# Wuziyi616/CFUN

Measured on AMD Instinct MI355X. Metric: volumes/sec fwd+bwd, 256x256x128 8-class CT, higher is better.
Workload: dtype f32; 1 GPU; cfg2: 256x256x128 CT, stage 'finetune', 4 positive + 8 negative RoIs, U-Net b=20, 96x96x96 crops -> 192x192x192 masks, 6 losses incl. 3-D Sobel edge loss, fwd+bwd; parallelism=single GPU

## Files before the change

cfun_amd/_lib.py:

```python
import ctypes as C
import os

import torch

_HERE = os.path.dirname(os.path.abspath(__file__))
DEFAULT_LIB = os.path.join(_HERE, "libcfun_hip.so")

ACT_NONE, ACT_RELU, ACT_LRELU = 0, 1, 2
ALGO_AUTO, ALGO_DIRECT, ALGO_MFMA = 0, 1, 2
ALGO_WINO = 4
ALGO_WINO2 = 5
TILE_G16, TILE_G8 = 0x100, 0x200


class ConvParams(C.Structure):
    _fields_ = [(n, C.c_int32) for n in ("N", "Di", "Hi", "Wi", "Ci", "Do", "Ho", "Wo", "Co", "CoP", "CiP",
                                         "kd", "kh", "kw", "stride", "pd", "ph", "pw", "up2", "act")] + \
               [("slope", C.c_float)] + \
               [(n, C.c_int32) for n in ("scale_mode", "has_shift", "res_mode", "res_up2", "d2s", "d2s_cq", "tap_skip", "algo",
                                         "w_prepared")]


class ConvFusion(C.Structure):
    _fields_ = [("in_stats", C.c_void_p), ("in_act", C.c_int32), ("in_slope", C.c_float), ("out_stats", C.c_void_p),
                ("out_eps", C.c_float)]


FUSE_OUT_STATS, FUSE_IN_NORM, FUSE_IN_NORM_WGRAD = 1, 2, 4


class WeightJob(C.Structure):
    _fields_ = [("w", C.c_void_p), ("fwd", C.c_void_p), ("dgrad", C.c_void_p), ("co_idx", C.c_void_p), ("ci_idx", C.c_void_p),
                ("Co", C.c_int32), ("Ci", C.c_int32), ("T", C.c_int32), ("src_ci", C.c_int32), ("fwd_kind", C.c_int32),
                ("dgrad_kind", C.c_int32), ("block_begin", C.c_uint32), ("reserved", C.c_int32)]


WOP_NONE = 0

_P = C.c_void_p
_I = C.c_int32
_L = C.c_int64
_F = C.c_float
_Z = C.c_size_t
_PP = C.POINTER(ConvParams)
_PF = C.POINTER(ConvFusion)

_SIGNATURES = {
    "cfun_version": (C.c_int, []),
    "cfun_error_string": (C.c_char_p, [C.c_int]),
    "cfun_conv3d_fwd_workspace_bytes": (_Z, [_PP]),
    "cfun_conv3d_fwd_kernel": (_I, [_PP]),
    "cfun_conv3d_wino_plan": (C.c_int, [_PP, C.POINTER(C.c_int32)]),
    "cfun_conv3d_fwd": (C.c_int, [_P, _P, _P, _P, _P, _P, _PP, _P, _Z, _P]),
    "cfun_conv3d_fused_support": (C.c_int, [_PP]),
    "cfun_conv3d_fwd_fused_workspace_bytes": (_Z, [_PP, _PF]),
    "cfun_conv3d_fwd_fused": (C.c_int, [_P, _P, _P, _P, _P, _P, _PP, _PF, _P, _Z, _P]),
    "cfun_conv3d_bwd_weight_fused": (C.c_int, [_P, _P, _P, _I, _PP, _PF, _P, _Z, _P]),
    "cfun_conv3d_bwd_data_workspace_bytes": (_Z, [_PP]),
    "cfun_conv3d_bwd_data": (C.c_int, [_P, _P, _P, _PP, _P, _Z, _P]),
    "cfun_conv3d_bwd_weight_workspace_bytes": (_Z, [_PP]),
    "cfun_conv3d_bwd_weight": (C.c_int, [_P, _P, _P, _PP, _P, _Z, _P]),
    "cfun_conv3d_bwd_weight_oidhw": (C.c_int, [_P, _P, _P, _PP, _P, _Z, _P]),
    "cfun_act_bwd": (C.c_int, [_P, _P, _P, _P, _L, _I, _L, _I, _F, _I, _P]),
    "cfun_channel_sum_workspace_bytes": (_Z, [_L, _I]),
    "cfun_channel_sum": (C.c_int, [_P, _P, _L, _I, _P, _Z, _P]),
    "cfun_fc_workspace_bytes": (_Z, [_I, _I, _I]),
    "cfun_fc_fwd": (C.c_int, [_P, _P, _P, _P, _P, _I, _I, _I, _I, _P, _Z, _P]),
    "cfun_fc_bwd_weight": (C.c_int, [_P, _P, _P, _I, _I, _I, _P]),
    "cfun_fc_bwd_weight_max_rows": (_I, [_I]),
    "cfun_fc_bwd_data": (C.c_int, [_P, _P, _P, _I, _I, _I, _P]),
    "cfun_lrelu_fwd": (C.c_int, [_P, _P, _L, _F, _P]),
    "cfun_lrelu_bwd": (C.c_int, [_P, _P, _P, _L, _F, _P]),
    "cfun_add": (C.c_int, [_P, _P, _P, _L, _P]),
    "cfun_lrelu_bwd_add": (C.c_int, [_P, _P, _P, _P, _L, _I, _L, _F, _P]),
    "cfun_instnorm_lrelu_bwd_add": (C.c_int, [_P, _P, _P, _P, _P, _I, _L, _I, _L, _F, _P, _Z, _P]),
    "cfun_upsample2_bwd": (C.c_int, [_P, _P, _I, _I, _I, _I, _I, _P]),
    "cfun_instnorm_workspace_bytes": (_Z, [_I, _L, _I]),
    "cfun_instnorm_stats": (C.c_int, [_P, _P, _I, _L, _I, _F, _P, _Z, _P]),
    "cfun_instnorm_lrelu_fwd": (C.c_int, [_P, _P, _P, _I, _L, _I, _F, _P]),
    "cfun_instnorm_lrelu_bwd": (C.c_int, [_P, _P, _P, _P, _I, _L, _I, _F, _P, _Z, _P]),
    "cfun_instnorm_lrelu_fwd_strided": (C.c_int, [_P, _P, _P, _I, _L, _I, _L, _F, _P]),
    "cfun_instnorm_lrelu_bwd_strided": (C.c_int, [_P, _P, _P, _P, _I, _L, _I, _L, _F, _P, _Z, _P]),
    "cfun_instnorm_bwd_means": (C.c_int, [_P, _P, _P, _P, _I, _L, _I, _L, _F, _P, _Z, _P]),
    "cfun_instnorm_lrelu_bwd_apply": (C.c_int, [_P, _P, _P, _P, _P, _I, _L, _I, _L, _F, _P]),
    "cfun_lrelu_fwd_strided": (C.c_int, [_P, _P, _L, _I, _L, _L, _F, _P]),
    "cfun_lrelu_bwd_strided": (C.c_int, [_P, _P, _P, _L, _I, _L, _F, _P]),
    "cfun_maxpool2_fwd": (C.c_int, [_P, _P, _P, _I, _I, _I, _I, _I, _P]),
    "cfun_maxpool2_bwd": (C.c_int, [_P, _P, _P, _I, _I, _I, _I, _I, _P]),
    "cfun_roi_align3d_fwd": (C.c_int, [_P, _P, _P, _P, _I, _I, _I, _I, _I, _I, _I, _I, _P]),
    "cfun_roi_align3d_bwd": (C.c_int, [_P, _P, _P, _I, _I, _I, _I, _I, _I, _I, _I, _P]),
    "cfun_roi_align3d_slab_fwd": (C.c_int, [_P, _P, _P, _P, _I, _I, _I, _I, _I, _I, _I, _I, _I, _I, _P]),
    "cfun_roi_align3d_slab_bwd": (C.c_int, [_P, _P, _P, _I, _I, _I, _I, _I, _I, _I, _I, _I, _I, _P]),
    "cfun_nms3d_workspace_bytes": (_Z, [_I]),
    "cfun_nms3d": (C.c_int, [_P, _P, _I, _F, _I, _P, _P, _P, _Z, _P]),
    "cfun_softmax_fwd": (C.c_int, [_P, _P, _L, _I, _P]),
    "cfun_softmax_bwd": (C.c_int, [_P, _P, _P, _L, _I, _P]),
    "cfun_loss_workspace_bytes": (_Z, [_L]),
    "cfun_softmax_ce_fwd": (C.c_int, [_P, _P, _P, _L, _I, _P, _Z, _P]),
    "cfun_softmax_ce_bwd": (C.c_int, [_P, _P, _P, _P, _L, _I, _P]),
    "cfun_edge_loss_fwd": (C.c_int, [_P, _P, _P, _I, _I, _I, _I, _I, _P, _Z, _P]),
    "cfun_edge_loss_bwd_workspace_bytes": (_Z, [_I, _I, _I, _I, _I]),
    "cfun_edge_loss_bwd": (C.c_int, [_P, _P, _P, _P, _I, _I, _I, _I, _I, _P, _Z, _P]),
    "cfun_mask_losses_bwd": (C.c_int, [_P, _P, _P, _P, _P, _I, _I, _I, _I, _I, _P, _Z, _P]),
    "cfun_edge_loss_fwd_save": (C.c_int, [_P, _P, _P, _P, _I, _I, _I, _I, _I, _P, _Z, _P]),
    "cfun_mask_losses_bwd_saved": (C.c_int, [_P, _P, _P, _P, _P, _P, _I, _I, _I, _I, _I, _P]),
    "cfun_mask_fused_workspace_bytes": (_Z, []),
    "cfun_mask_fused_supported": (C.c_int, [_I, _I, _I, _I, _I]),
    "cfun_mask_fused_fwd": (C.c_int, [_P, _P, _P, _P, _P, _I, _I, _I, _I, _I, _P, _Z, _P]),
    "cfun_mask_fused_u_bytes": (_Z, [_I, _I, _I, _I, _I]),
    "cfun_mask_fused_bwd": (C.c_int, [_P, _P, _P, _P, _P, _I, _I, _I, _I, _I, _P]),
    "cfun_mask_target_labels": (C.c_int, [_P, _P, _P, _I, _I, _I, _I, _I, _I, _I, _P]),
    "cfun_ce_weighted_workspace_bytes": (_Z, []),
    "cfun_softmax_ce_weighted_fwd": (C.c_int, [_P, _P, _P, _P, _P, _L, _I, _P, _Z, _P]),
    "cfun_softmax_ce_weighted_bwd": (C.c_int, [_P, _P, _P, _P, _P, _P, _L, _I, _P]),
    "cfun_edge_raw_dc_bytes": (_Z, [_I, _I, _I, _I, _I]),
    "cfun_edge_raw_fwd": (C.c_int, [_P, _P, _P, _P, _I, _I, _I, _I, _I, _P, _Z, _P]),
    "cfun_edge_raw_bwd": (C.c_int, [_P, _P, _P, _I, _I, _I, _I, _I, _P]),
    "cfun_unmold_argmax": (C.c_int, [_P, _P, _I, _I, _I, _I, _I, _I, _I, _P, _P]),
    "cfun_unmold_overlap": (C.c_int, [_P, _P, _I, _P, _P, _I, _I, _I, _I, _I, _I, _I, _P]),
    "cfun_sumsq_partials_count": (C.c_int32, []),
    "cfun_sumsq_partials": (C.c_int, [_P, C.c_int64, _P, _P]),
    "cfun_norm_finalize": (C.c_int, [_P, _I, _P, _P]),
    "cfun_sgd_momentum_step": (C.c_int, [_P, _P, _P, C.c_int64, C.c_float, C.c_float, C.c_float, C.c_float, _P, _I, _P]),
    "cfun_weight_pack": (C.c_int, [_P, _P, _I, _I, _I, _P]),
    "cfun_weight_pack_transpose": (C.c_int, [_P, _P, _I, _I, _I, _P]),
    "cfun_weight_pack_both": (C.c_int, [_P, _P, _P, _I, _I, _I, _P]),
    "cfun_fold_up2_fwd": (C.c_int, [_P, _P, _I, _I, _I, _I, _P]),
    "cfun_fold_up2_bwd": (C.c_int, [_P, _P, _I, _I, _I, _I, _P]),
    "cfun_weight_prepare_kinds": (C.c_int, [_PP, C.POINTER(C.c_int32), C.POINTER(C.c_size_t)]),
    "cfun_weight_prepare_plan": (C.c_int, [C.POINTER(WeightJob), _I, C.POINTER(C.c_int64)]),
    "cfun_weight_prepare": (C.c_int, [_P, _I, _L, _P]),
    "cfun_weight_unpack": (C.c_int, [_P, _P, _I, _I, _I, _P]),
    "cfun_halo_pack": (C.c_int, [_P, _P, _I, _I, _I, _I, _I, _I, _I, _P]),
    "cfun_halo_unpack": (C.c_int, [_P, _P, _I, _I, _I, _I, _I, _I, _I, _P]),
    "cfun_resize3d": (C.c_int, [_P, _P, _P, _P, _P, _P, _P, _I, _P, _P]),
}

EXPORTS = tuple(_SIGNATURES)

_D = C.c_double
SAMPLE_SIGNATURES = {
    "cfun_sample_workspace_bytes": (_Z, [_I, _I, _I, _I, _I]),
    "cfun_sample_rotate_bbox": (C.c_int, [_P, _P, _P, _P, _P, _D, _D, _I, _P, _P, _P, _P, _P, _P, _Z, _P]),
    "cfun_sample_rpn_targets": (C.c_int, [_P, _I, _P, _I, _P, _I, _P, _D, _D, _P, _P, _P, _P, _Z, _P]),
}
SAMPLE_EXPORTS = tuple(SAMPLE_SIGNATURES)

TILE_SIGNATURES = {
    "cfun_conv3d_fwd_tile": (C.c_int, [_PP, C.POINTER(C.c_int32)]),
}
TILE_EXPORTS = tuple(TILE_SIGNATURES)

EVAL_SIGNATURES = {
    "cfun_seg_confusion_workspace_bytes": (_Z, [_I, _I, _I, _I]),
    "cfun_seg_confusion": (C.c_int, [_P, _P, _I, _P, _P, _I, _P, _P, _Z, _P]),
}
EVAL_EXPORTS = tuple(EVAL_SIGNATURES)

CC_CLASS, CC_FOREGROUND = 0, 1
CC_SIGNATURES = {
    "cfun_cc_workspace_bytes": (_Z, [_I, _I, _I, _I]),
    "cfun_cc_label": (C.c_int, [_P, _P, _I, _I, _P, _P, _Z, _P]),
    "cfun_cc_filter": (C.c_int, [_P, _P, _P, _I, _I, _I, _L, _P, _P, _P, _Z, _P]),
}
CC_EXPORTS = tuple(CC_SIGNATURES)

_lib = None
_lib_path = None
_is_emulator = False


def lib_path():
    return os.environ.get("CFUN_LIB_PATH") or DEFAULT_LIB


def load():
    global _lib, _lib_path, _is_emulator
    path = lib_path()
    if _lib is not None and _lib_path == path:
        return _lib
    if not os.path.exists(path):
        raise RuntimeError(
            "cfun_amd: %s not found -- the HIP library is required (no CPU fallback). Build it with "
            "`make -C cfun_amd/csrc -j8` or `python -c 'import __graft_entry__ as g; g.build()'`." % path)
    lib = C.CDLL(path)
    for name, (res, args) in list(_SIGNATURES.items()) + list(SAMPLE_SIGNATURES.items()) + list(TILE_SIGNATURES.items()) + \
            list(EVAL_SIGNATURES.items()) + list(CC_SIGNATURES.items()):
        fn = getattr(lib, name)
        fn.restype = res
        fn.argtypes = args
    _lib, _lib_path = lib, path
    _is_emulator = os.path.basename(path).startswith("libcfun_emu")
    return lib


def is_emulator():
    load()
    return _is_emulator


def check(rc, what):
    if rc != 0:
        msg = load().cfun_error_string(rc)
        raise RuntimeError("cfun_amd: %s failed (%d): %s" % (what, rc, msg.decode() if msg else "?"))


def ptr(t):
    if t is None:
        return None
    if not t.is_contiguous():
        raise RuntimeError("cfun_amd: kernel argument must be contiguous, got strides %s" % (t.stride(),))
    if not t.is_cuda and not is_emulator():
        raise RuntimeError("cfun_amd: CPU tensor passed to a HIP kernel (there is no CPU fallback)")
    return t.data_ptr()


def stream(t):
    if t.is_cuda:
        return torch.cuda.current_stream(t.device).cuda_stream
    return None


def workspace(nbytes, like):
    return torch.empty(max(int(nbytes), 256), dtype=torch.uint8, device=like.device)
```

cfun_amd/csrc/conv3d.hip:

```cpp
#include <stdlib.h>

#include "conv3d_mfma.h"
#include "../../include/cfun_tile.h"

int cfun_conv_fwd_direct(const float*, const float*, const float*, const float*, const float*, float*,
                         const CfunConv3dParams*, hipStream_t);
int cfun_conv_bwd_data_direct(const float*, const float*, float*, const CfunConv3dParams*, hipStream_t);
int cfun_conv_bwd_weight_direct(const float*, const float*, CfunWgradDst, const CfunConv3dParams*, void*, size_t, hipStream_t);
size_t cfun_direct_wgrad_ws(const CfunConv3dParams*);
int cfun_wgrad_finish(const float*, CfunWgradDst, const CfunConv3dParams*, int, hipStream_t);
int cfun_wgrad_zero(CfunWgradDst, const CfunConv3dParams*, hipStream_t);
int cfun_conv_stem_supported(const CfunConv3dParams*);
int cfun_conv_stem_fwd(const float*, const float*, const float*, const float*, float*, const CfunConv3dParams*, hipStream_t);
int cfun_conv_pointwise_supported(const CfunConv3dParams*);
int cfun_conv_pointwise_in_supported(const CfunConv3dParams*);
int cfun_conv_pointwise_fwd(const float*, const float*, const float*, const float*, const float*, float*,
                            const CfunConv3dParams*, const float*, int, float, hipStream_t);
int cfun_wino_supported(const CfunConv3dParams*);
size_t cfun_wino_workspace_bytes(const CfunConv3dParams*);
int cfun_wino_s2d_dgrad_supported(const CfunConv3dParams*, const CfunConv3dParams*);
int cfun_wino_fwd(const float*, const float*, int, int, const float*, const float*, const float*, float*,
                  const CfunConv3dParams*, void*, size_t, const cfun_mfma::ConvMode*, int, hipStream_t);
int cfun_wino_is_2d(const CfunConv3dParams*);
int cfun_wino_geom(const CfunConv3dParams*);
int cfun_wino_stat_slots(const CfunConv3dParams*, size_t);
int cfun_stats_finalize(const double* part, float* stats, int N, int slots, int C, int64_t V, float eps, int slot_minor, hipStream_t st);
int cfun_wino_wgrad_supported(const CfunConv3dParams*);
size_t cfun_wino_wgrad_workspace_bytes(const CfunConv3dParams*);
int cfun_wino_wgrad(const float*, const float*, float*, const CfunConv3dParams*, int*, hipStream_t);
int cfun_wgrad_c1_supported(const CfunConv3dParams*);
size_t cfun_wgrad_c1_ws(const CfunConv3dParams*);
int cfun_wgrad_c1(const float*, const float*, CfunWgradDst, const CfunConv3dParams*, void*, size_t, hipStream_t);

namespace {

typedef int (*FwdFn)(int, const float*, const float*, const float*, const float*, const float*, float*,
                     const CfunConv3dParams&, const cfun_mfma::ConvMode&, void*, size_t, hipStream_t);
typedef size_t (*FwdWsFn)(int, const CfunConv3dParams&, const cfun_mfma::ConvMode&);
typedef void (*PlanFn)(const CfunConv3dParams&, int, cfun_mfma::WgPlan*);
typedef int (*WgFn)(const float*, const float*, float*, const CfunConv3dParams&, const cfun_mfma::WgPlan&, hipStream_t);

struct Shape {
  int kd, kh, kw, s;
  FwdFn fwd;
  FwdWsFn fwd_ws;
  PlanFn plan;
  WgFn wgrad;
  int max_nsub;
  FwdFn fwd8;
  FwdWsFn fwd_ws8;
};

#define SHAPE(NAME, KD, KH, KW, S, MAXN) \
  { KD, KH, KW, S, cfun_mfma_fwd_##NAME, cfun_mfma_fwd_ws_##NAME, cfun_mfma_wgrad_plan_##NAME, cfun_mfma_wgrad_##NAME, MAXN, \
    nullptr, nullptr }
#define SHAPE_G8(NAME, KD, KH, KW, S, MAXN) \
  { KD, KH, KW, S, cfun_mfma_fwd_##NAME, cfun_mfma_fwd_ws_##NAME, cfun_mfma_wgrad_plan_##NAME, cfun_mfma_wgrad_##NAME, MAXN, \
    cfun_mfma_fwd_g8_##NAME, cfun_mfma_fwd_ws_g8_##NAME }
const Shape kShapes[] = {
    SHAPE_G8(k333s1, 3, 3, 3, 1, 5), SHAPE_G8(k333s2, 3, 3, 3, 2, 5), SHAPE(k111s1, 1, 1, 1, 1, 5),
    SHAPE(k111s2, 1, 1, 1, 2, 5), SHAPE(k133s1, 1, 3, 3, 1, 5), SHAPE(k311s1, 3, 1, 1, 1, 5),
    SHAPE(k555s1, 5, 5, 5, 1, 1), SHAPE_G8(k222s1, 2, 2, 2, 1, 5),
};

const Shape* find_shape(int kd, int kh, int kw, int s) {
  for (const Shape& sh : kShapes)
    if (sh.kd == kd && sh.kh == kh && sh.kw == kw && sh.s == s) return &sh;
  return nullptr;
}

using cfun_mfma::ConvMode;
const ConvMode kPlain = {0, 0, 0, 0, 0, nullptr, 0, 0.f, nullptr, 0};

int pick_nsub_parity(int cqp, int max_nsub) {
  for (int n = max_nsub; n >= 1; --n)
    if (cqp % (16 * n) == 0) return n;
  return 0;
}

int pick_nsub(int co, int max_nsub) {
  int best = 1, best_pad = 1 << 30;
  for (int n = 1; n <= max_nsub; ++n) {
    const int nt = 16 * n;
    const int pad = (co + nt - 1) / nt * nt;
    if (pad <= best_pad) { best_pad = pad; best = n; }
  }
  return best;
}

bool standard_dims(const CfunConv3dParams* p) {
  const int sh = p->up2 ? 1 : 0;
  return (((p->Di << sh) + 2 * p->pd - p->kd) / p->stride + 1) == p->Do &&
         (((p->Hi << sh) + 2 * p->ph - p->kh) / p->stride + 1) == p->Ho &&
         (((p->Wi << sh) + 2 * p->pw - p->kw) / p->stride + 1) == p->Wo;
}

bool valid_params(const CfunConv3dParams* p) {
  if (!p) return false;
  if (p->N < 0 || p->Ci <= 0 || p->Co <= 0 || p->kd <= 0 || p->kh <= 0 || p->kw <= 0) return false;
  if (p->stride != 1 && p->stride != 2) return false;
  if (p->CoP < p->Co || (p->CoP & 15) || p->CiP < p->Ci || (p->CiP & 15)) return false;
  if (!standard_dims(p)) return false;
  if (p->d2s) {
    if ((p->Co & 7) || p->up2 || p->d2s_cq < 0 || p->d2s_cq > (p->Co >> 3)) return false;
    if (p->tap_skip && !(p->kd == 3 && p->kh == 3 && p->kw == 3 && p->stride == 1)) return false;
  } else if (p->tap_skip || p->d2s_cq) {
    return false;
  } else if (p->res_mode && p->res_up2 && ((p->Do | p->Ho | p->Wo) & 1)) {
    return false;
  }
  return true;
}

const Shape* mfma_shape(const CfunConv3dParams* p) {
  if ((p->Ci & 3) || (p->Co & 3)) return nullptr;
  if (p->d2s) {
    const int cqp = p->Co >> 3, cq = p->d2s_cq > 0 ? p->d2s_cq : cqp;
    if ((cqp & 3) || (cq & 3)) return nullptr;
    if (p->tap_skip && pick_nsub_parity(cqp, 5) == 0) return nullptr;
  }
  const Shape* s = find_shape(p->kd, p->kh, p->kw, p->stride);
  if (!s) return nullptr;
  if (p->Co > 16 * s->max_nsub && s->max_nsub == 1) return nullptr;
  return s;
}

int tile_geom_knob() {
  static int v = -2;
  if (v == -2) {
    const char* e = getenv("CFUN_TILE_GEOM");
    v = !e ? -1 : atoi(e) == 16 ? 0 : atoi(e) == 8 ? 1 : -1;
  }
  return v;
}

bool tile_geom_rule(const CfunConv3dParams* p) {
  using cfun_mfma::cdiv;
  const int64_t g16 = (int64_t)cdiv(p->Ho, 4) * 4 * cdiv(p->Wo, 16) * 16, g8 = (int64_t)cdiv(p->Ho, 8) * 8 * cdiv(p->Wo, 8) * 8;
  return g8 < g16;
}

bool make_dgrad_params(const CfunConv3dParams* p, CfunConv3dParams* q) {
  if (p->stride != 1 || !standard_dims(p)) return false;
  const int sh = p->up2 ? 1 : 0;
  *q = *p;
  q->Di = p->Do; q->Hi = p->Ho; q->Wi = p->Wo; q->Ci = p->Co;
  q->Do = p->Di << sh; q->Ho = p->Hi << sh; q->Wo = p->Wi << sh; q->Co = p->Ci;
  q->CoP = p->CiP; q->CiP = p->CoP;
  q->pd = p->kd - 1 - p->pd; q->ph = p->kh - 1 - p->ph; q->pw = p->kw - 1 - p->pw;
  if (q->pd < 0 || q->ph < 0 || q->pw < 0) return false;
  q->up2 = 0; q->act = CFUN_ACT_NONE; q->scale_mode = 0; q->has_shift = 0; q->res_mode = 0; q->res_up2 = 0;
  q->d2s = 0; q->d2s_cq = 0; q->tap_skip = 0; q->w_prepared = 0;
  return true;
}

bool use_folded_s2_dgrad(const CfunConv3dParams* p) {
  return CFUN_ALGO_OF(p->algo) != CFUN_ALGO_DIRECT && p->stride == 2 && !p->up2 && p->kd == 3 && p->kh == 3 && p->kw == 3 &&
         p->pd == 1 && p->ph == 1 && p->pw == 1 && !((p->Di | p->Hi | p->Wi) & 1) && !(p->Ci & 3) && !(p->Co & 3) &&
         p->Di == 2 * p->Do && p->Hi == 2 * p->Ho && p->Wi == 2 * p->Wo;
}

__global__ void __launch_bounds__(256)
k_fold_s2_dgrad_weights(const float* __restrict__ wpT, float* __restrict__ wd, int Ci, int Co, int CiP, int CoPd) {
  const int64_t total = (int64_t)8 * Co * CoPd;
  const int64_t i = (int64_t)blockIdx.x * 256 + threadIdx.x;
  if (i >= total) return;
  const int col = (int)(i % CoPd);
  const int co = (int)((i / CoPd) % Co);
  const int tap = (int)(i / ((int64_t)CoPd * Co));
  float v = 0.f;
  if (col < 8 * Ci) {
    const int q = col / Ci, ci = col - q * Ci;
    const int par[3] = {q >> 2, (q >> 1) & 1, q & 1}, off[3] = {tap >> 2, (tap >> 1) & 1, tap & 1};
    int t[3];
    bool ok = true;
    for (int d = 0; d < 3; ++d) {
      if (par[d] == 0) { t[d] = 1; ok = ok && off[d] == 0; }
      else t[d] = off[d] == 0 ? 2 : 0;
    }
    if (ok) v = wpT[((int64_t)((t[0] * 3 + t[1]) * 3 + t[2]) * Co + co) * CiP + ci];
  }
  wd[i] = v;
}

CfunConv3dParams folded_s2_params(const CfunConv3dParams* p) {
  CfunConv3dParams q = *p;
  q.Di = p->Do; q.Hi = p->Ho; q.Wi = p->Wo; q.Ci = p->Co;
  q.Do = p->Do; q.Ho = p->Ho; q.Wo = p->Wo; q.Co = 8 * p->Ci;
  q.CoP = (8 * p->Ci + 15) / 16 * 16; q.CiP = p->CoP;
  q.kd = q.kh = q.kw = 2; q.stride = 1; q.pd = q.ph = q.pw = 0;
  q.up2 = 0; q.act = CFUN_ACT_NONE; q.scale_mode = 0; q.has_shift = 0; q.res_mode = 0; q.res_up2 = 0; q.d2s = 1;
  q.d2s_cq = 0; q.tap_skip = 0; q.w_prepared = 0;
  return q;
}

int wgrad_max_nsub(const Shape* s) {
  static int cap = -1;
  if (cap < 0) {
    const char* e = getenv("CFUN_WGRAD_MAX_NSUB");
    cap = e ? atoi(e) : 5;
    if (cap < 1 || cap > 5) cap = 5;
  }
  return s->max_nsub < cap ? s->max_nsub : cap;
}

int wgrad_nsub(const CfunConv3dParams* p, const Shape* s) {
  if (p->d2s && p->tap_skip) {
    const int cqp = p->Co >> 3, mx = wgrad_max_nsub(s);
    const int tiles = (cqp + 16 * mx - 1) / (16 * mx);
    return (cqp + 16 * tiles - 1) / (16 * tiles);
  }
  return pick_nsub(p->CoP, wgrad_max_nsub(s));
}

bool use_mfma_dgrad(const CfunConv3dParams* p, CfunConv3dParams* q, const Shape** s) {
  if (CFUN_ALGO_OF(p->algo) == CFUN_ALGO_DIRECT) return false;
  if (!make_dgrad_params(p, q)) return false;
  *s = mfma_shape(q);
  return *s != nullptr;
}

__global__ void __launch_bounds__(256)
k_splitk_finish(const float4* __restrict__ partial, int ksplit, const float* __restrict__ scale,
                const float* __restrict__ shift, const float* __restrict__ res, float4* __restrict__ y,
                CfunConv3dParams p, int64_t total4) {
  const int C4 = p.Co >> 2;
  for (int64_t i = (int64_t)blockIdx.x * 256 + threadIdx.x; i < total4; i += (int64_t)gridDim.x * 256) {
    float4 a = partial[i];
    for (int k = 1; k < ksplit; ++k) {
      const float4 b = partial[(int64_t)k * total4 + i];
      a.x += b.x; a.y += b.y; a.z += b.z; a.w += b.w;
    }
    const int64_t v = i / C4;
    const int co = (int)(i - v * C4) * 4;
    if (p.scale_mode) {
      const int64_t n = v / ((int64_t)p.Do * p.Ho * p.Wo);
      const float4 s4 = *reinterpret_cast<const float4*>(scale + (p.scale_mode == 2 ? n * p.Co : 0) + co);
      a.x *= s4.x; a.y *= s4.y; a.z *= s4.z; a.w *= s4.w;
    }
    if (p.has_shift) {
      const float4 t = *reinterpret_cast<const float4*>(shift + co);
      a.x += t.x; a.y += t.y; a.z += t.z; a.w += t.w;
    }
    if (p.res_mode) {
      int64_t rv = v;
      if (p.res_up2) {
        int64_t t = v;
        const int ox = (int)(t % p.Wo); t /= p.Wo;
        const int oy = (int)(t % p.Ho); t /= p.Ho;
        const int oz = (int)(t % p.Do);
        const int64_t n = t / p.Do;
        rv = ((n * (p.Do >> 1) + (oz >> 1)) * (p.Ho >> 1) + (oy >> 1)) * (p.Wo >> 1) + (ox >> 1);
      }
      const float4 t4 = *reinterpret_cast<const float4*>(res + rv * p.Co + co);
      a.x += t4.x; a.y += t4.y; a.z += t4.z; a.w += t4.w;
    }
    a.x = cfun_apply_act(a.x, p.act, p.slope); a.y = cfun_apply_act(a.y, p.act, p.slope);
    a.z = cfun_apply_act(a.z, p.act, p.slope); a.w = cfun_apply_act(a.w, p.act, p.slope);
    y[i] = a;
  }
}

__global__ void __launch_bounds__(256)
k_splitk_finish_stats(const float4* __restrict__ partial, int ksplit, const float* __restrict__ scale,
                      const float* __restrict__ shift, const float* __restrict__ res, float4* __restrict__ y,
                      CfunConv3dParams p, int64_t V, int lanes, double* __restrict__ part) {
  __shared__ double sm[256 * 8];
  const int C4 = p.Co >> 2, tid = threadIdx.x;
  const int cg = tid % C4, vl = tid / C4, n = blockIdx.y, co = cg * 4;
  const int64_t total4 = (int64_t)p.N * V * C4;
  double acc[2][4] = {{0.0, 0.0, 0.0, 0.0}, {0.0, 0.0, 0.0, 0.0}};
  if (vl < lanes) {
    float4 s4 = make_float4(1.f, 1.f, 1.f, 1.f), t4 = make_float4(0.f, 0.f, 0.f, 0.f);
    if (p.scale_mode) s4 = *reinterpret_cast<const float4*>(scale + (p.scale_mode == 2 ? n * p.Co : 0) + co);
    if (p.has_shift) t4 = *reinterpret_cast<const float4*>(shift + co);
#pragma unroll 4
    for (int64_t vv = (int64_t)blockIdx.x * lanes + vl; vv < V; vv += (int64_t)gridDim.x * lanes) {
      const int64_t v = (int64_t)n * V + vv, i = v * C4 + cg;
      float4 a = partial[i];
      for (int k = 1; k < ksplit; ++k) {
        const float4 b = partial[(int64_t)k * total4 + i];
        a.x += b.x; a.y += b.y; a.z += b.z; a.w += b.w;
      }
      if (p.scale_mode) { a.x *= s4.x; a.y *= s4.y; a.z *= s4.z; a.w *= s4.w; }
      if (p.has_shift) { a.x += t4.x; a.y += t4.y; a.z += t4.z; a.w += t4.w; }
      if (p.res_mode) {
        int64_t rv = v;
        if (p.res_up2) {
          int64_t t = vv;
          const int ox = (int)(t % p.Wo); t /= p.Wo;
          const int oy = (int)(t % p.Ho);
          const int oz = (int)(t / p.Ho);
          rv = (((int64_t)n * (p.Do >> 1) + (oz >> 1)) * (p.Ho >> 1) + (oy >> 1)) * (p.Wo >> 1) + (ox >> 1);
        }
        const float4 r4 = *reinterpret_cast<const float4*>(res + rv * p.Co + co);
        a.x += r4.x; a.y += r4.y; a.z += r4.z; a.w += r4.w;
      }
      a.x = cfun_apply_act(a.x, p.act, p.slope); a.y = cfun_apply_act(a.y, p.act, p.slope);
      a.z = cfun_apply_act(a.z, p.act, p.slope); a.w = cfun_apply_act(a.w, p.act, p.slope);
      y[i] = a;
      acc[0][0] += a.x; acc[0][1] += a.y; acc[0][2] += a.z; acc[0][3] += a.w;
      acc[1][0] += (double)a.x * a.x; acc[1][1] += (double)a.y * a.y; acc[1][2] += (double)a.z * a.z; acc[1][3] += (double)a.w * a.w;
    }
  }
#pragma unroll
  for (int q = 0; q < 2; ++q)
#pragma unroll
    for (int j = 0; j < 4; ++j) sm[(tid * 2 + q) * 4 + j] = acc[q][j];
  __syncthreads();
  if (vl == 0) {
    for (int l = 1; l < lanes; ++l) {
      const int t2 = l * C4 + cg;
#pragma unroll
      for (int q = 0; q < 2; ++q)
#pragma unroll
        for (int j = 0; j < 4; ++j) acc[q][j] += sm[(t2 * 2 + q) * 4 + j];
    }
    double* out = part + ((int64_t)n * gridDim.x + blockIdx.x) * 2 * p.Co;
#pragma unroll
    for (int q = 0; q < 2; ++q)
#pragma unroll
      for (int j = 0; j < 4; ++j) out[(int64_t)q * p.Co + co + j] = acc[q][j];
  }
}

int splitk_stats_blocks(const CfunConv3dParams* p, int* lanes_out) {
  const int C4 = p->Co >> 2;
  if ((p->Co & 3) || C4 > 256 || C4 < 1) return 0;
  const int lanes = 256 / C4;
  const int64_t V = (int64_t)p->Do * p->Ho * p->Wo;
  int64_t want = (4096 + p->N - 1) / (p->N > 0 ? p->N : 1);
  int64_t maxb = (V + (int64_t)lanes * 4 - 1) / ((int64_t)lanes * 4);
  if (maxb < 1) maxb = 1;
  if (lanes_out) *lanes_out = lanes;
  return (int)(want < maxb ? want : maxb);
}

}

int cfun_splitk_stat_slots(const CfunConv3dParams* p) { return splitk_stats_blocks(p, nullptr); }

int cfun_tile_geom(const CfunConv3dParams* p, int g8_exists) {
  if (!g8_exists || (p->algo & CFUN_ALGO_TILE_G16)) return 0;
  if (p->algo & CFUN_ALGO_TILE_G8) return 1;
  if (tile_geom_knob() >= 0) return tile_geom_knob();
  return g8_exists == 1 && tile_geom_rule(p) ? 1 : 0;
}

int cfun_splitk_finish(const float* partial, int ksplit, const float* scale, const float* shift, const float* res,
                       float* y, const CfunConv3dParams* p, double* stat_part, hipStream_t st) {
  if (stat_part) {
    int lanes = 0;
    const int blocks = splitk_stats_blocks(p, &lanes);
    if (blocks <= 0) return CFUN_EINVAL;
    hipLaunchKernelGGL(k_splitk_finish_stats, dim3((unsigned)blocks, (unsigned)p->N), dim3(256), 0, st, (const float4*)partial,
                       ksplit, scale, shift, res, (float4*)y, *p, (int64_t)p->Do * p->Ho * p->Wo, lanes, stat_part);
    CFUN_LAUNCH_CHECK();
    return CFUN_OK;
  }
  const int64_t total4 = (int64_t)p->N * p->Do * p->Ho * p->Wo * (p->Co >> 2);
  int64_t blocks = (total4 + 255) / 256;
  if (blocks > 2048) blocks = 2048;
  hipLaunchKernelGGL(k_splitk_finish, dim3((unsigned)blocks), dim3(256), 0, st, (const float4*)partial, ksplit, scale, shift,
                     res, (float4*)y, *p, total4);
  CFUN_LAUNCH_CHECK();
  return CFUN_OK;
}

extern "C" {

int cfun_version(void) { return CFUN_VERSION; }

const char* cfun_error_string(int code) {
  switch (code) {
    case CFUN_OK: return "ok";
    case CFUN_EINVAL: return "cfun: invalid argument or unsupported shape";
    case CFUN_EWORKSPACE: return "cfun: workspace too small";
    case CFUN_EALIGN: return "cfun: pointer not 16-byte aligned";
    default: return code > 0 ? hipGetErrorString((hipError_t)code) : "cfun: unknown error";
  }
}

static int pick_tile(const Shape* s, int co, bool per_parity) {
  const bool rem_ok = (s->kd == 3 && s->kh == 3 && s->kw == 3) || (s->kd == 1 && s->kh == 1 && s->kw == 1 && s->s == 1);
  if (rem_ok && s->max_nsub > 1) {
    if (co == 20) return 1 + 8 * 1;
    if (co == 8 && s->kd == 3) return 0 + 8 * 2;
  }
  return per_parity ? pick_nsub_parity(co, s->max_nsub) : pick_nsub(co, s->max_nsub);
}

static void fwd_mode(const CfunConv3dParams* p, const Shape* s, ConvMode* md, int* nsub) {
  *md = kPlain;
  *nsub = pick_tile(s, p->Co, false);
  if (p->d2s && p->tap_skip) {
    md->tap_skip = 1;
    *nsub = pick_tile(s, p->Co >> 3, true);
  }
}

static bool g8_loses_wave(const Shape* s, const ConvMode& md, int nsub) {
  if (s->kd == 2) return nsub == 1;
  if (s->s == 2) return nsub == 1 || nsub == 4 || nsub == 0 + 8 * 2;
  if (md.tap_skip == 1 || md.in_s2d) return false;
  return nsub == 3 || nsub == 4 || nsub == 5 || nsub == 1 + 8 * 1;
}

static bool g8_no_gain(const CfunConv3dParams* p, const Shape* s, const ConvMode& md) {
  return (s->kd == 2 || md.tap_skip == 1) && (int64_t)p->Do * p->Ho * p->Wo <= 6 * 6 * 6;
}

static int mfma_geom(const CfunConv3dParams* p, const Shape* s, const ConvMode& md, int nsub) {
  const bool has = s->fwd8 && nsub != 2 + 8 * 2 && (!md.in_s2d || (md.tap_skip == 2 && nsub < 8));
  return cfun_tile_geom(p, !has ? 0 : (g8_loses_wave(s, md, nsub) || g8_no_gain(p, s, md)) ? 2 : 1);
}

size_t cfun_conv3d_fwd_workspace_bytes(const CfunConv3dParams* p) {
  if (!valid_params(p)) return 0;
  const Shape* s = CFUN_ALGO_OF(p->algo) == CFUN_ALGO_DIRECT ? nullptr : mfma_shape(p);
  if (!s) return 256;
  ConvMode md;
  int nsub;
  fwd_mode(p, s, &md, &nsub);
  size_t need = (mfma_geom(p, s, md, nsub) ? s->fwd_ws8 : s->fwd_ws)(nsub, *p, md);
  if (cfun_wino_supported(p) && cfun_wino_workspace_bytes(p) > need) need = cfun_wino_workspace_bytes(p);
  return cfun_align_up(need + 256, 256);
}

int cfun_conv3d_fwd_kernel(const CfunConv3dParams* p);

int cfun_conv3d_fwd_tile(const CfunConv3dParams* p, int32_t out[3]) {
  if (!out || !valid_params(p)) return CFUN_EINVAL;
  const int k = cfun_conv3d_fwd_kernel(p);
  if (k != CFUN_KERNEL_MFMA && k != CFUN_KERNEL_WINO) return CFUN_EINVAL;
  int g;
  if (k == CFUN_KERNEL_WINO) {
    g = cfun_wino_geom(p);
  } else {
    ConvMode md;
    int nsub;
    const Shape* s = mfma_shape(p);
    fwd_mode(p, s, &md, &nsub);
    g = mfma_geom(p, s, md, nsub);
  }
  out[0] = 4; out[1] = g ? 8 : 4; out[2] = g ? 8 : 16;
  return CFUN_OK;
}

int cfun_conv3d_fwd_kernel(const CfunConv3dParams* p) {
  if (!valid_params(p)) return CFUN_EINVAL;
  if (CFUN_ALGO_OF(p->algo) == CFUN_ALGO_AUTO && cfun_conv_pointwise_supported(p)) return CFUN_KERNEL_POINTWISE;
  if (CFUN_ALGO_OF(p->algo) != CFUN_ALGO_DIRECT && mfma_shape(p)) return cfun_wino_supported(p) ? CFUN_KERNEL_WINO : CFUN_KERNEL_MFMA;
  if (CFUN_ALGO_OF(p->algo) != CFUN_ALGO_DIRECT && CFUN_ALGO_OF(p->algo) != CFUN_ALGO_MFMA && cfun_conv_stem_supported(p)) return CFUN_KERNEL_STEM;
  return CFUN_KERNEL_DIRECT;
}

static int conv_fwd_impl(const float* x, const float* wp, const float* scale, const float* shift, const float* res,
                         float* y, const CfunConv3dParams* p, const ConvMode* fz, void* ws, size_t ws_bytes,
                         int* stat_slots, cfun_stream_t stream) {
  if (!valid_params(p)) return CFUN_EINVAL;
  if ((p->scale_mode && !scale) || (p->has_shift && !shift) || (p->res_mode && !res)) return CFUN_EINVAL;
  if (p->scale_mode < 0 || p->scale_mode > 2 || p->res_mode < 0 || p->res_mode > 1) return CFUN_EINVAL;
  const bool fused = fz && (fz->in_stats || fz->in_act || fz->out_part);
  if (CFUN_ALGO_OF(p->algo) == CFUN_ALGO_AUTO && cfun_conv_pointwise_supported(p) && cfun_aligned16(x) && cfun_aligned16(y)) {
    if (fused && (fz->out_part || !cfun_conv_pointwise_in_supported(p))) return CFUN_EINVAL;
    return cfun_conv_pointwise_fwd(x, wp, scale, shift, res, y, p, fused ? fz->in_stats : nullptr, fused ? fz->in_act : 0,
                                   fused ? fz->in_slope : 0.f, cfun_st(stream));
  }
  const Shape* s = CFUN_ALGO_OF(p->algo) == CFUN_ALGO_DIRECT ? nullptr : mfma_shape(p);
  if (s) {
    if (!cfun_aligned16(x) || !cfun_aligned16(wp) || !cfun_aligned16(y) || (scale && !cfun_aligned16(scale)) ||
        (shift && !cfun_aligned16(shift)) || (res && !cfun_aligned16(res)))
      return CFUN_EALIGN;
    ConvMode md;
    int nsub;
    fwd_mode(p, s, &md, &nsub);
    if (fused) { md.in_stats = fz->in_stats; md.in_act = fz->in_act; md.in_slope = fz->in_slope; md.out_part = fz->out_part; }
    if (ws && !cfun_aligned16(ws)) return CFUN_EALIGN;
    const bool prepared = (p->w_prepared & 1) != 0;
    if (ws && cfun_wino_supported(p) && ws_bytes >= cfun_wino_workspace_bytes(p)) {
      if (md.in_stats || md.in_act) return CFUN_EINVAL;
      if (stat_slots) *stat_slots = cfun_wino_stat_slots(p, ws_bytes);
      return cfun_wino_fwd(x, wp, 0, 0, scale, shift, res, y, p, ws, ws_bytes, &md, prepared, cfun_st(stream));
    }
    if (prepared && cfun_wino_supported(p)) return CFUN_EWORKSPACE;
    const int geom = mfma_geom(p, s, md, nsub);
    if (stat_slots) *stat_slots = cfun_mfma::fwd_stat_slots(nsub, geom, *p, md, ws ? ws_bytes : 0);
    return (geom ? s->fwd8 : s->fwd)(nsub, x, wp, scale, shift, res, y, *p, md, ws, ws ? ws_bytes : 0, cfun_st(stream));
  }
  if (fused) return CFUN_EINVAL;
  if (CFUN_ALGO_OF(p->algo) == CFUN_ALGO_MFMA) return CFUN_EINVAL;
  if (CFUN_ALGO_OF(p->algo) != CFUN_ALGO_DIRECT && cfun_conv_stem_supported(p) && cfun_aligned16(y))
    return cfun_conv_stem_fwd(x, wp, scale, shift, y, p, cfun_st(stream));
  return cfun_conv_fwd_direct(x, wp, scale, shift, res, y, p, cfun_st(stream));
}

int cfun_conv3d_fwd(const float* x, const float* wp, const float* scale, const float* shift, const float* res,
                    float* y, const CfunConv3dParams* p, void* ws, size_t ws_bytes, cfun_stream_t stream) {
  return conv_fwd_impl(x, wp, scale, shift, res, y, p, nullptr, ws, ws_bytes, nullptr, stream);
}

static bool wgrad_takes_prologue(const CfunConv3dParams* p);

int cfun_conv3d_fused_support(const CfunConv3dParams* p) {
  if (!valid_params(p) || CFUN_ALGO_OF(p->algo) == CFUN_ALGO_DIRECT || !mfma_shape(p)) return 0;
  const int wg = wgrad_takes_prologue(p) ? CFUN_FUSE_IN_NORM_WGRAD : 0;
  if (CFUN_ALGO_OF(p->algo) == CFUN_ALGO_AUTO && cfun_conv_pointwise_supported(p))
    return cfun_conv_pointwise_in_supported(p) ? (CFUN_FUSE_IN_NORM | wg) : 0;
  const int st = (p->Co >> 2) <= 256 ? CFUN_FUSE_OUT_STATS : 0;
  if (cfun_wino_supported(p)) return st;
  return st | CFUN_FUSE_IN_NORM | wg;
}

static size_t stat_part_bytes(const CfunConv3dParams* p) {
  using cfun_mfma::cdiv;
  const int t16 = cdiv(p->Do, 4) * cdiv(p->Ho, 4) * cdiv(p->Wo, 16), t8 = cdiv(p->Do, 4) * cdiv(p->Ho, 8) * cdiv(p->Wo, 8);
  const int tiles = (t16 > t8 ? t16 : t8) * (p->d2s ? 8 : 1);
  const int sk = cfun_splitk_stat_slots(p);
  const int cy = p->d2s ? (p->d2s_cq > 0 ? p->d2s_cq : (p->Co >> 3)) : p->Co;
  return cfun_align_up((size_t)p->N * (tiles > sk ? tiles : sk) * 2 * cy * sizeof(double), 256);
}

size_t cfun_conv3d_fwd_fused_workspace_bytes(const CfunConv3dParams* p, const CfunConvFusion* f) {
  const size_t main_bytes = cfun_conv3d_fwd_workspace_bytes(p);
  if (!main_bytes || !f || !f->out_stats) return main_bytes;
  return main_bytes + stat_part_bytes(p);
}

int cfun_conv3d_fwd_fused(const float* x, const float* wp, const float* scale, const float* shift, const float* res,
                          float* y, const CfunConv3dParams* p, const CfunConvFusion* f, void* ws, size_t ws_bytes,
                          cfun_stream_t stream) {
  if (!f || (!f->in_stats && !f->in_act && !f->out_stats))
    return conv_fwd_impl(x, wp, scale, shift, res, y, p, nullptr, ws, ws_bytes, nullptr, stream);
  const int have = cfun_conv3d_fused_support(p);
  const int want = (f->out_stats ? CFUN_FUSE_OUT_STATS : 0) | ((f->in_stats || f->in_act) ? CFUN_FUSE_IN_NORM : 0);
  if ((want & have) != want) return CFUN_EINVAL;
  if (f->in_act != CFUN_ACT_NONE && (f->in_act != CFUN_ACT_LRELU || f->in_slope < 0.f || f->in_slope > 1.f)) return CFUN_EINVAL;
  ConvMode fz = kPlain;
  fz.in_stats = f->in_stats;
  fz.in_act = (f->in_stats || f->in_act) ? CFUN_ACT_LRELU : CFUN_ACT_NONE;
  fz.in_slope = f->in_act == CFUN_ACT_LRELU ? f->in_slope : 1.f;
  const size_t main_bytes = cfun_conv3d_fwd_workspace_bytes(p);
  if (f->out_stats) {
    if (!ws || !cfun_aligned16(ws) || ws_bytes < main_bytes + stat_part_bytes(p)) return CFUN_EWORKSPACE;
    fz.out_part = (double*)((char*)ws + main_bytes);
  }
  int slots = 0;
  const int rc = conv_fwd_impl(x, wp, scale, shift, res, y, p, &fz, ws, f->out_stats ? main_bytes : ws_bytes, &slots, stream);
  if (rc || !f->out_stats) return rc;
  if (slots == 0) return CFUN_EINVAL;
  const int cy = p->d2s ? (p->d2s_cq > 0 ? p->d2s_cq : (p->Co >> 3)) : p->Co;
  return cfun_stats_finalize(fz.out_part, f->out_stats, p->N, slots < 0 ? -slots : slots, cy,
                             (int64_t)p->Do * p->Ho * p->Wo * (p->d2s ? 8 : 1), f->out_eps, slots > 0, cfun_st(stream));
}

int cfun_weight_prepare_kinds(const CfunConv3dParams* p, int32_t kinds[2], size_t bytes[2]) {
  if (!kinds || !bytes) return CFUN_EINVAL;
  kinds[0] = kinds[1] = CFUN_WOP_NONE;
  bytes[0] = bytes[1] = 0;
  if (!valid_params(p)) return CFUN_EINVAL;
  const int T = p->kd * p->kh * p->kw;
  if (T > 27) return CFUN_OK;
  kinds[0] = CFUN_WOP_PACK;
  bytes[0] = (size_t)T * p->Ci * p->CoP * sizeof(float);
  const bool pointwise = CFUN_ALGO_OF(p->algo) == CFUN_ALGO_AUTO && cfun_conv_pointwise_supported(p);
  if (!pointwise && CFUN_ALGO_OF(p->algo) != CFUN_ALGO_DIRECT && mfma_shape(p) && cfun_wino_supported(p)) {
    const int twod = cfun_wino_is_2d(p);
    kinds[0] = twod ? CFUN_WOP_WINO2 : CFUN_WOP_WINO1;
    bytes[0] = (size_t)(twod ? 48 : 36) * p->Ci * p->CoP * sizeof(float);
  }
  kinds[1] = CFUN_WOP_PACKT;
  bytes[1] = (size_t)T * p->Co * p->CiP * sizeof(float);
  CfunConv3dParams q;
  const Shape* s;
  if (use_folded_s2_dgrad(p)) {
    kinds[1] = CFUN_WOP_S2FOLD;
    bytes[1] = (size_t)8 * p->Co * ((8 * p->Ci + 15) / 16 * 16) * sizeof(float);
  } else if (use_mfma_dgrad(p, &q, &s) && !p->up2 &&
             (p->d2s ? cfun_wino_s2d_dgrad_supported(p, &q) : cfun_wino_supported(&q))) {
    const int twod = cfun_wino_is_2d(&q);
    kinds[1] = twod ? CFUN_WOP_WINO2_T : CFUN_WOP_WINO1_T;
    bytes[1] = (size_t)(twod ? 48 : 36) * p->Co * p->CiP * sizeof(float);
  }
  return CFUN_OK;
}

size_t cfun_conv3d_bwd_data_workspace_bytes(const CfunConv3dParams* p) {
  if (!valid_params(p)) return 0;
  CfunConv3dParams q;
  const Shape* s;
  if (use_folded_s2_dgrad(p)) return cfun_align_up((size_t)8 * p->Co * ((8 * p->Ci + 15) / 16 * 16) * sizeof(float), 256);
  if (use_mfma_dgrad(p, &q, &s)) {
    if (p->up2) return cfun_align_up((size_t)q.N * q.Do * q.Ho * q.Wo * q.Co * sizeof(float), 256);
    ConvMode md = kPlain;
    md.flip = 1;
    if (p->d2s) { md.in_s2d = 1; md.in_cqp = p->Co >> 3; md.in_cq = p->d2s_cq > 0 ? p->d2s_cq : md.in_cqp; }
    const int nsub = pick_tile(s, q.Co, false);
    if (p->d2s) md.tap_skip = p->tap_skip ? 2 : 0;
    size_t need = (mfma_geom(&q, s, md, nsub) ? s->fwd_ws8 : s->fwd_ws)(nsub, q, md);
    if ((p->d2s ? cfun_wino_s2d_dgrad_supported(p, &q) : cfun_wino_supported(&q)) && cfun_wino_workspace_bytes(&q) > need)
      need = cfun_wino_workspace_bytes(&q);
    return cfun_align_up(need + 256, 256);
  }
  return 256;
}

int cfun_conv3d_bwd_data(const float* g, const float* wpT, float* dx, const CfunConv3dParams* p, void* ws,
                         size_t ws_bytes, cfun_stream_t stream) {
  if (!valid_params(p)) return CFUN_EINVAL;
  CfunConv3dParams q;
  const Shape* s;
  const bool prepared = (p->w_prepared & 2) != 0;
  if (use_folded_s2_dgrad(p)) {
    if (!cfun_aligned16(g) || !cfun_aligned16(wpT) || !cfun_aligned16(dx) || !cfun_aligned16(ws)) return CFUN_EALIGN;
    if (ws_bytes < cfun_conv3d_bwd_data_workspace_bytes(p)) return CFUN_EWORKSPACE;
    q = folded_s2_params(p);
    const float* wd = wpT;
    if (!prepared) {
      const int64_t nw = (int64_t)8 * p->Co * q.CoP;
      hipLaunchKernelGGL(k_fold_s2_dgrad_weights, dim3((unsigned)((nw + 255) / 256)), dim3(256), 0, cfun_st(stream), wpT,
                         (float*)ws, p->Ci, p->Co, p->CiP, q.CoP);
      CFUN_LAUNCH_CHECK();
      wd = (const float*)ws;
    }
    const Shape* s2 = find_shape(2, 2, 2, 1);
    const int nsub = pick_nsub(q.Co, s2->max_nsub);
    return (mfma_geom(&q, s2, kPlain, nsub) ? s2->fwd8 : s2->fwd)(nsub, g, wd, nullptr, nullptr, nullptr, dx, q, kPlain, nullptr, 0,
                                                                   cfun_st(stream));
  }
  if (use_mfma_dgrad(p, &q, &s)) {
    if (!cfun_aligned16(g) || !cfun_aligned16(wpT) || !cfun_aligned16(dx)) return CFUN_EALIGN;
    const int nsub = pick_tile(s, q.Co, false);
    ConvMode md = kPlain;
    md.flip = 1;
    if (p->d2s) {
      md.in_s2d = 1;
      md.in_cqp = p->Co >> 3;
      md.in_cq = p->d2s_cq > 0 ? p->d2s_cq : md.in_cqp;
      md.tap_skip = p->tap_skip ? 2 : 0;
    }
    const bool wino = !p->up2 && (p->d2s ? cfun_wino_s2d_dgrad_supported(p, &q) : cfun_wino_supported(&q));
    if (wino && cfun_aligned16(ws) && ws_bytes >= cfun_wino_workspace_bytes(&q))
      return cfun_wino_fwd(g, wpT, 1, p->d2s ? (p->Co >> 3) : 0, nullptr, nullptr, nullptr, dx, &q, ws, ws_bytes, nullptr,
                           prepared, cfun_st(stream));
    if (wino && prepared) return CFUN_EWORKSPACE;
    const FwdFn fwd = mfma_geom(&q, s, md, nsub) ? s->fwd8 : s->fwd;
    if (!p->up2) return fwd(nsub, g, wpT, nullptr, nullptr, nullptr, dx, q, md, ws, cfun_aligned16(ws) ? ws_bytes : 0, cfun_st(stream));
    if (ws_bytes < cfun_conv3d_bwd_data_workspace_bytes(p) || !cfun_aligned16(ws)) return CFUN_EWORKSPACE;
    const int rc = fwd(nsub, g, wpT, nullptr, nullptr, nullptr, (float*)ws, q, md, nullptr, 0, cfun_st(stream));
    if (rc) return rc;
    return cfun_upsample2_bwd((const float*)ws, dx, p->N, p->Di, p->Hi, p->Wi, p->Ci, stream);
  }
  return cfun_conv_bwd_data_direct(g, wpT, dx, p, cfun_st(stream));
}

static bool wgrad_mfma_fits(const CfunConv3dParams* p) {
  const int64_t lim = (int64_t)1 << 31;
  const int64_t go = (int64_t)p->N * p->Do * p->Ho * p->Wo * p->Co;
  return (int64_t)p->N * p->Di * p->Hi * p->Wi * p->Ci < lim && go < lim;
}

size_t cfun_conv3d_bwd_weight_workspace_bytes(const CfunConv3dParams* p) {
  if (!valid_params(p)) return 0;
  if (CFUN_ALGO_OF(p->algo) != CFUN_ALGO_DIRECT && cfun_wgrad_c1_supported(p)) return cfun_align_up(cfun_wgrad_c1_ws(p), 256);
  const Shape* s = (CFUN_ALGO_OF(p->algo) == CFUN_ALGO_DIRECT || !wgrad_mfma_fits(p)) ? nullptr : mfma_shape(p);
  if (s && cfun_wino_wgrad_supported(p)) return cfun_align_up(cfun_wino_wgrad_workspace_bytes(p), 256);
  if (s) {
    cfun_mfma::WgPlan w;
    s->plan(*p, wgrad_nsub(p, s), &w);
    return cfun_align_up((size_t)w.nchunks * w.kslots * p->kd * p->kh * p->kw * p->Ci * p->CoP * sizeof(float), 256);
  }
  return cfun_align_up(cfun_direct_wgrad_ws(p), 256);
}

static bool wgrad_takes_prologue(const CfunConv3dParams* p) {
  if (CFUN_ALGO_OF(p->algo) == CFUN_ALGO_DIRECT || !wgrad_mfma_fits(p) || !mfma_shape(p)) return false;
  return !cfun_wgrad_c1_supported(p) && !cfun_wino_wgrad_supported(p);
}

static int bwd_weight_any(const float* x, const float* g, CfunWgradDst dst, const CfunConv3dParams* p,
                          const CfunConvFusion* f, void* ws, size_t ws_bytes, cfun_stream_t stream) {
  if (!valid_params(p)) return CFUN_EINVAL;
  const bool pro = f && (f->in_stats || f->in_act);
  if (pro && !wgrad_takes_prologue(p)) return CFUN_EINVAL;
  if (CFUN_ALGO_OF(p->algo) != CFUN_ALGO_DIRECT && cfun_wgrad_c1_supported(p) && (int64_t)p->N * p->Do * p->Ho * p->Wo > 0) {
    if (!cfun_aligned16(g) || !cfun_aligned16(ws)) return CFUN_EALIGN;
    return cfun_wgrad_c1(x, g, dst, p, ws, ws_bytes, cfun_st(stream));
  }
  const Shape* s = (CFUN_ALGO_OF(p->algo) == CFUN_ALGO_DIRECT || !wgrad_mfma_fits(p)) ? nullptr : mfma_shape(p);
  if (s) {
    if (!cfun_aligned16(x) || !cfun_aligned16(g)) return CFUN_EALIGN;
    if (ws_bytes < cfun_conv3d_bwd_weight_workspace_bytes(p)) return CFUN_EWORKSPACE;
    if (cfun_wino_wgrad_supported(p)) {
      if (!cfun_aligned16(ws)) return CFUN_EALIGN;
      int nparts = 0;
      const int rc = cfun_wino_wgrad(x, g, (float*)ws, p, &nparts, cfun_st(stream));
      if (rc) return rc;
      return cfun_wgrad_finish((const float*)ws, dst, p, nparts, cfun_st(stream));
    }
    cfun_mfma::WgPlan w;
    s->plan(*p, wgrad_nsub(p, s), &w);
    if (pro) {
      if (f->in_act != CFUN_ACT_NONE && (f->in_act != CFUN_ACT_LRELU || f->in_slope < 0.f || f->in_slope > 1.f)) return CFUN_EINVAL;
      w.in_stats = f->in_stats; w.in_act = CFUN_ACT_LRELU; w.in_slope = f->in_act == CFUN_ACT_LRELU ? f->in_slope : 1.f;
    }
    if (w.ntiles == 0) return cfun_wgrad_zero(dst, p, cfun_st(stream));
    const int rc = s->wgrad(x, g, (float*)ws, *p, w, cfun_st(stream));
    if (rc) return rc;
    return cfun_wgrad_finish((const float*)ws, dst, p, w.nchunks * w.kslots, cfun_st(stream));
  }
  if (CFUN_ALGO_OF(p->algo) == CFUN_ALGO_MFMA) return CFUN_EINVAL;
  return cfun_conv_bwd_weight_direct(x, g, dst, p, ws, ws_bytes, cfun_st(stream));
}

int cfun_conv3d_bwd_weight(const float* x, const float* g, float* dwp, const CfunConv3dParams* p, void* ws,
                           size_t ws_bytes, cfun_stream_t stream) {
  return bwd_weight_any(x, g, CfunWgradDst{dwp, 0}, p, nullptr, ws, ws_bytes, stream);
}

int cfun_conv3d_bwd_weight_oidhw(const float* x, const float* g, float* dw, const CfunConv3dParams* p, void* ws,
                                 size_t ws_bytes, cfun_stream_t stream) {
  return bwd_weight_any(x, g, CfunWgradDst{dw, 1}, p, nullptr, ws, ws_bytes, stream);
}

int cfun_conv3d_bwd_weight_fused(const float* x, const float* g, float* dw, int32_t oidhw, const CfunConv3dParams* p,
                                 const CfunConvFusion* f, void* ws, size_t ws_bytes, cfun_stream_t stream) {
  return bwd_weight_any(x, g, CfunWgradDst{dw, oidhw ? 1 : 0}, p, f, ws, ws_bytes, stream);
}

}
```

cfun_amd/csrc/conv3d_mfma.h:

```cpp
#pragma once
#include <type_traits>

#include "common.h"

typedef float f32x4 __attribute__((ext_vector_type(4)));

int cfun_splitk_finish(const float* partial, int ksplit, const float* scale, const float* shift, const float* res,
                       float* y, const CfunConv3dParams* p, double* stat_part, hipStream_t st);
int cfun_splitk_stat_slots(const CfunConv3dParams* p);

namespace cfun_mfma {

constexpr int pad_plane(int v, int rs, int g = 0) { return rs != 1 ? (v | 1) : v + (((g ? 8 : 16) - (v % 32)) + 32) % 32; }
constexpr int pad_row16(int v) { return (v % 32 == 16) ? v : v + 16; }
constexpr int cdiv(int a, int b) { return (a + b - 1) / b; }
constexpr int row_stride(int nt) { return nt <= 16 ? 16 : nt <= 48 ? 48 : nt <= 80 ? 80 : pad_row16((nt + 15) / 16 * 16); }

__device__ __forceinline__ unsigned xcd_remap(unsigned bid, unsigned nwg) {
  const unsigned q = nwg >> 3, r = nwg & 7u, xcd = bid & 7u, local = bid >> 3;
  const unsigned base = xcd < r ? xcd * (q + 1) : r * (q + 1) + (xcd - r) * q;
  return base + local;
}

__device__ __forceinline__ void tile_raster(unsigned t, int ntz, int nty, int ntx, int& tz, int& ty, int& tx) {
  constexpr int SZ = 4, SY = 4;
  const unsigned band = (unsigned)(SZ * nty * ntx);
  const int zb = (int)(t / band);
  unsigned r = t - (unsigned)zb * band;
  const int bz = ntz - zb * SZ < SZ ? ntz - zb * SZ : SZ;
  const unsigned sup = (unsigned)(bz * SY * ntx);
  const int yb = (int)(r / sup);
  r -= (unsigned)yb * sup;
  const int by = nty - yb * SY < SY ? nty - yb * SY : SY;
  const int tzi = (int)(r / (unsigned)(by * ntx));
  r -= (unsigned)(tzi * by * ntx);
  tz = zb * SZ + tzi;
  ty = yb * SY + (int)(r / (unsigned)ntx);
  tx = (int)(r % (unsigned)ntx);
}

struct ConvMode {
  int flip;
  int in_s2d;
  int in_cq, in_cqp;
  int tap_skip;
  const float* in_stats;
  int in_act;
  float in_slope;
  double* out_part;
  int out_slots;
};

__device__ __forceinline__ float norm_act_in(float v, float mean, float rstd, int, float slope) {
  const float xh = (v - mean) * rstd;
  return fmaxf(xh, xh * slope);
}
__device__ __forceinline__ float4 norm_act_in4(const float4& v, const float4& s01, const float4& s23, int act, float slope) {
  return make_float4(norm_act_in(v.x, s01.x, s01.y, act, slope), norm_act_in(v.y, s01.z, s01.w, act, slope),
                     norm_act_in(v.z, s23.x, s23.y, act, slope), norm_act_in(v.w, s23.z, s23.w, act, slope));
}

constexpr int STAT_ROUND = 32;
constexpr int stat_es(int chans) { return 2 * chans + 8; }
constexpr int stat_lds_floats(int nt) { return 64 * stat_es(nt < STAT_ROUND ? nt : STAT_ROUND); }
__device__ __forceinline__ void quad_park_16(const float (&sa)[4], const float (&sb)[4], float* red, int es, int wv, int lane, int cl) {
  float* r = red + (wv * 16 + (lane & 15)) * es + (cl + (lane >> 4) * 4) * 2;
  *reinterpret_cast<float4*>(r) = make_float4(sa[0], sb[0], sa[1], sb[1]);
  *reinterpret_cast<float4*>(r + 4) = make_float4(sa[2], sb[2], sa[3], sb[3]);
}
__device__ __forceinline__ void quad_park_wave(const float (&sa)[4], const float (&sb)[4], float* red, int es, int wv, int lane, int cl) {
  float u[4], v[4];
#pragma unroll
  for (int j = 0; j < 4; ++j) {
    u[j] = sa[j]; v[j] = sb[j];
    u[j] += __shfl_xor(u[j], 16, 64); v[j] += __shfl_xor(v[j], 16, 64);
    u[j] += __shfl_xor(u[j], 32, 64); v[j] += __shfl_xor(v[j], 32, 64);
  }
  if ((lane >> 4) == 0) {
    float* r = red + (wv * 16 + (lane & 15)) * es + cl * 2;
    *reinterpret_cast<float4*>(r) = make_float4(u[0], v[0], u[1], v[1]);
    *reinterpret_cast<float4*>(r + 4) = make_float4(u[2], v[2], u[3], v[3]);
  }
}
__device__ __forceinline__ void stat_round_flush(const float* red, int es, int tid, int c0, int nch, int cobase, int n, int tile,
                                                 const CfunConv3dParams& p, const ConvMode& md) {
  __syncthreads();
  if (tid < 2 * nch) {
    const int cl = tid >> 1, qn = tid & 1, co = cobase + c0 + cl;
    if (co < p.Co) {
      double sum = 0.0;
#pragma unroll 8
      for (int e = 0; e < 64; ++e) sum += (double)red[e * es + cl * 2 + qn];
      int slot = tile, ch = co, cy = p.Co;
      if (p.d2s) {
        const int CqP = p.Co >> 3;
        cy = p.d2s_cq > 0 ? p.d2s_cq : CqP;
        const int q = co / CqP;
        ch = co - q * CqP;
        slot = tile * 8 + q;
      }
      if (ch < cy) md.out_part[(((int64_t)n * 2 + qn) * cy + ch) * md.out_slots + slot] = sum;
    }
  }
  __syncthreads();
}

__device__ __forceinline__ unsigned parity_tapmask(int q, bool flip) {
  unsigned m = 0;
  const int pz = q >> 2, py = (q >> 1) & 1, px = q & 1;
  for (int dz = pz; dz <= pz + 1; ++dz)
    for (int dy = py; dy <= py + 1; ++dy)
      for (int dx = px; dx <= px + 1; ++dx) {
        const int tap = (dz * 3 + dy) * 3 + dx;
        m |= 1u << (flip ? 26 - tap : tap);
      }
  return m;
}

template <int KD, int KH, int KW, int S, int G = 0>
struct FwdTile {
  static constexpr int TD = 4, TH = G ? 8 : 4, TW = G ? 8 : 16;
  static constexpr int MR = 16 / TW;
  static constexpr int TAPS = KD * KH * KW;
  static constexpr bool COMPACT = TAPS == 1;
  static constexpr int RS = COMPACT ? 1 : S;
  static constexpr int IZ = COMPACT ? TD : (TD - 1) * S + KD;
  static constexpr int IY = COMPACT ? TH : (TH - 1) * S + KH;
  static constexpr int IX = COMPACT ? TW : (TW - 1) * S + KW;
  static constexpr int IVOX = IZ * IY * IX;
  static constexpr int IXS = (G == 0 || COMPACT) ? IX : (RS == 1 ? 16 : 24);
  static_assert(IX <= IXS && (G == 0 || COMPACT || (RS * IXS) % 32 == 16), "G8 row stride");
  static constexpr int PLANEP = pad_plane(IZ * IY * IXS, RS, G);
  static constexpr int PASS = IXS == IX ? 256 : (256 / IX) * IX;
  static constexpr int IN_LOADS = cdiv(IVOX, PASS);
};

template <int NSUB, int MODE, int REM, bool STATS, int G>
constexpr int conv_min_waves() { return (G == 1 && MODE == 2 && !STATS && REM == 0) ? (NSUB == 2 ? 5 : NSUB == 3 ? 4 : 1) : 1; }

template <int KD, int KH, int KW, int S, int NSUB, int MODE, int REM, bool STATS = false, int G = 0>
__global__ void __launch_bounds__(256, (conv_min_waves<NSUB, MODE, REM, STATS, G>()))
k_conv_mfma(const float* __restrict__ x, const float* __restrict__ wp, const float* __restrict__ scale,
            const float* __restrict__ shift, const float* __restrict__ res, float* __restrict__ y,
            CfunConv3dParams p, ConvMode md, int ntz, int nty, int ntx, int ncot, float* __restrict__ partial,
            int chunks_per_split) {
  constexpr bool SPECIAL = MODE != 0, UPF = MODE == 2, UPD = MODE == 3;
  static_assert(!UPD || (KD == 3 && KH == 3 && KW == 3 && S == 1 && NSUB > 0 && REM == 0), "up-conv data-gradient tiles");
  static_assert(!UPF || (KD == 3 && KH == 3 && KW == 3 && S == 1 && NSUB > 0 && REM == 0), "up-conv forward tiles");
  using T = FwdTile<KD, KH, KW, S, G>;
  constexpr int TAPS = T::TAPS, NT = 16 * NSUB + 4 * REM, NTP = row_stride(NT), NS1 = NSUB > 0 ? NSUB : 1;
  constexpr int W_ITEMS = TAPS * NT;
  constexpr int W_LOADS = cdiv(W_ITEMS, 256);
  CFUN_DYN_LDS(float, smem);
  float* Xl = smem;
  float* Wl = smem + 4 * T::PLANEP;

  const int tid = threadIdx.x, lane = tid & 63, wv = __builtin_amdgcn_readfirstlane(tid >> 6);
  unsigned lid = xcd_remap(blockIdx.x, gridDim.x);
  const int cot = lid % ncot; lid /= ncot;
  const unsigned per_n = (unsigned)(ntz * nty * ntx);
  const int n = lid / per_n;
  int tz, ty, tx;
  tile_raster(lid - (unsigned)n * per_n, ntz, nty, ntx, tz, ty, tx);
  const int z0 = tz * T::TD, y0 = ty * T::TH, x0 = tx * T::TW;
  const int cobase = cot * NT;
  const int sh = p.up2 ? 1 : 0;
  const int Dv = p.Di << sh, Hv = p.Hi << sh, Wv = p.Wi << sh;

  int64_t in_off[T::IN_LOADS];
#pragma unroll
  for (int i = 0; i < T::IN_LOADS; ++i) {
    const int idx = tid + i * T::PASS;
    in_off[i] = -1;
    if (tid < T::PASS && idx < T::IVOX) {
      const int ix = idx % T::IX, iy = (idx / T::IX) % T::IY, iz = idx / (T::IX * T::IY);
      int vz, vy, vx;
      if (T::COMPACT) { vz = (z0 + iz) * S - p.pd; vy = (y0 + iy) * S - p.ph; vx = (x0 + ix) * S - p.pw; }
      else { vz = z0 * S - p.pd + iz; vy = y0 * S - p.ph + iy; vx = x0 * S - p.pw + ix; }
      if (vz >= 0 && vz < Dv && vy >= 0 && vy < Hv && vx >= 0 && vx < Wv) {
        if (SPECIAL && md.in_s2d)
          in_off[i] = ((((int64_t)n * 2 * p.Di + 2 * vz) * 2 * p.Hi + 2 * vy) * 2 * p.Wi + 2 * vx) * md.in_cq;
        else
          in_off[i] = ((((int64_t)n * p.Di + (vz >> sh)) * p.Hi + (vy >> sh)) * p.Wi + (vx >> sh)) * p.Ci;
      }
    }
  }
  const int xl0 = T::IXS == T::IX ? tid : (tid / T::IX) * T::IXS + tid % T::IX;
  const int cpq = (SPECIAL && md.in_s2d) ? (md.in_cq >> 2) : 1;
  auto chunk_xoff = [&](int c) -> int64_t {
    if (!SPECIAL || !md.in_s2d) return (int64_t)c * 4;
    const int q = c / cpq, o4 = c - q * cpq;
    return ((int64_t)((q >> 2) * 2 * p.Hi + ((q >> 1) & 1)) * 2 * p.Wi + (q & 1)) * md.in_cq + o4 * 4;
  };
  auto chunk_wrow = [&](int c) -> int {
    if (!SPECIAL || !md.in_s2d) return c * 4;
    const int q = c / cpq, o4 = c - q * cpq;
    return q * md.in_cqp + o4 * 4;
  };
  float4 xin[T::IN_LOADS], win[W_LOADS];
  const int w_items = (UPF || (SPECIAL && TAPS == 27 && md.tap_skip)) ? 8 * NT : W_ITEMS;
  const int CqPw = p.Co >> 3;
  int q_staged = 0;
  auto live_tap_of = [](int q, int j) {
    return (((q >> 2) + (j >> 2)) * 3 + (((q >> 1) & 1) + ((j >> 1) & 1))) * 3 + ((q & 1) + (j & 1));
  };
  const bool in_fused = md.in_stats != nullptr || md.in_act != CFUN_ACT_NONE;
  float4 ns01 = make_float4(0.f, 1.f, 0.f, 1.f), ns23 = make_float4(0.f, 1.f, 0.f, 1.f);
  auto prefetch = [&](int c) {
    const int64_t xo = chunk_xoff(c);
    const int wrow = chunk_wrow(c);
    if (md.in_stats) {
      const float4* sp = reinterpret_cast<const float4*>(md.in_stats + ((int64_t)n * p.Ci + c * 4) * 2);
      ns01 = sp[0]; ns23 = sp[1];
    }
#pragma unroll
    for (int i = 0; i < T::IN_LOADS; ++i)
      xin[i] = in_off[i] >= 0 ? *reinterpret_cast<const float4*>(x + in_off[i] + xo) : make_float4(0.f, 0.f, 0.f, 0.f);
    if (SPECIAL && TAPS == 27 && md.tap_skip == 2) q_staged = c / cpq;
#pragma unroll
    for (int i = 0; i < W_LOADS; ++i) {
      const int it = tid + i * 256;
      win[i] = make_float4(0.f, 0.f, 0.f, 0.f);
      if (it < w_items) {
        const int row = it / (NT / 4), col = (it % (NT / 4)) * 4;
        int tapw = row >> 2;
        const int cc = row & 3;
        if (UPF) tapw = live_tap_of((cobase + col) / CqPw, tapw);
        else if (SPECIAL && TAPS == 27 && md.tap_skip) tapw = live_tap_of(q_staged, tapw);
        else if (md.flip) tapw = TAPS - 1 - tapw;
        if (cobase + col < p.CoP)
          win[i] = *reinterpret_cast<const float4*>(wp + ((int64_t)tapw * p.Ci + wrow + cc) * p.CoP + cobase + col);
      }
    }
  };
  auto commit = [&]() {
    if (in_fused) {
#pragma unroll
      for (int i = 0; i < T::IN_LOADS; ++i)
        if (in_off[i] >= 0) xin[i] = norm_act_in4(xin[i], ns01, ns23, md.in_act, md.in_slope);
    }
#pragma unroll
    for (int i = 0; i < T::IN_LOADS; ++i) {
      const int idx = tid + i * T::PASS;
      if (tid < T::PASS && idx < T::IVOX) {
        const int l = T::IXS == T::IX ? idx : xl0 + i * (T::PASS / T::IX) * T::IXS;
        Xl[l] = xin[i].x; Xl[T::PLANEP + l] = xin[i].y;
        Xl[2 * T::PLANEP + l] = xin[i].z; Xl[3 * T::PLANEP + l] = xin[i].w;
      }
    }
#pragma unroll
    for (int i = 0; i < W_LOADS; ++i) {
      const int it = tid + i * 256;
      if (it < w_items) {
        int row = it / (NT / 4);
        const int col = (it % (NT / 4)) * 4;
        if (!UPD && SPECIAL && TAPS == 27 && md.tap_skip == 2) {
          const int t = live_tap_of(q_staged, row >> 2);
          row = (md.flip ? TAPS - 1 - t : t) * 4 + (row & 3);
        }
        *reinterpret_cast<float4*>(Wl + row * NTP + col) = win[i];
      }
    }
  };

  f32x4 acc[4][NS1], accr[REM > 0 ? REM : 1];
#pragma unroll
  for (int m = 0; m < 4; ++m)
#pragma unroll
    for (int nn = 0; nn < NS1; ++nn) acc[m][nn] = f32x4{0.f, 0.f, 0.f, 0.f};
#pragma unroll
  for (int q = 0; q < (REM > 0 ? REM : 1); ++q) accr[q] = f32x4{0.f, 0.f, 0.f, 0.f};

  const int mrow = (lane & 15) / T::TW, mx = (lane & 15) % T::TW;
  const float* Xw = Xl + (lane >> 4) * T::PLANEP + (wv * T::RS * T::IY + mrow * T::RS) * T::IXS + mx * T::RS;
  const float* Ww = Wl + (lane >> 4) * NTP + (lane & 15);
  const float* Xr = Xl + ((wv * T::RS) * T::IY + (lane / T::TW) * T::RS) * T::IXS + (lane % T::TW) * T::RS;
  const float* Wr = Wl + 16 * NSUB + (lane & 3);

  const int nchunks = (SPECIAL && md.in_s2d) ? 8 * cpq : (p.Ci >> 2);
  const int CqP = p.Co >> 3;
  unsigned tapmask = 0xffffffffu;
  const int c_begin = blockIdx.y * chunks_per_split;
  const int c_end = (c_begin + chunks_per_split < nchunks) ? c_begin + chunks_per_split : nchunks;
  if (c_begin < c_end) prefetch(c_begin);
  for (int c = c_begin; c < c_end; ++c) {
    __syncthreads();
    commit();
    __syncthreads();
    if (c + 1 < c_end) prefetch(c + 1);
    if (SPECIAL && TAPS == 27 && md.tap_skip == 2) tapmask = parity_tapmask(c / cpq, true);
    if constexpr (UPF) {
#pragma unroll
      for (int nn = 0; nn < NSUB; ++nn) {
        const int q = (cobase + nn * 16) / CqP;
        const float* xq = Xw + (((q >> 2) * T::IY + ((q >> 1) & 1)) * T::IXS + (q & 1));
#pragma unroll
        for (int j = 0; j < 8; ++j) {
          const float a = Ww[j * 4 * NTP + nn * 16];
          const float* xt = xq + (((j >> 2) * T::IY + ((j >> 1) & 1)) * T::IXS + (j & 1));
#pragma unroll
          for (int m = 0; m < 4; ++m)
            acc[m][nn] = __builtin_amdgcn_mfma_f32_16x16x4f32(a, xt[m * T::MR * T::RS * T::IXS], acc[m][nn], 0, 0, 0);
        }
#ifndef CFUN_HIP_EMULATION
        __builtin_amdgcn_sched_barrier(0);
#endif
      }
    } else if constexpr (UPD) {
      const int q = c / cpq;
      const float* xq = Xw + (((2 - (q >> 2)) * T::IY + (2 - ((q >> 1) & 1))) * T::IXS + (2 - (q & 1)));
#pragma unroll
      for (int j = 0; j < 8; ++j) {
        float a[NS1];
#pragma unroll
        for (int nn = 0; nn < NSUB; ++nn) a[nn] = Ww[j * 4 * NTP + nn * 16];
        const float* xt = xq - (((j >> 2) * T::IY + ((j >> 1) & 1)) * T::IXS + (j & 1));
#pragma unroll
        for (int m = 0; m < 4; ++m) {
          const float b = xt[m * T::MR * T::RS * T::IXS];
#pragma unroll
          for (int nn = 0; nn < NSUB; ++nn) acc[m][nn] = __builtin_amdgcn_mfma_f32_16x16x4f32(a[nn], b, acc[m][nn], 0, 0, 0);
        }
#ifndef CFUN_HIP_EMULATION
        if (j & 1) __builtin_amdgcn_sched_barrier(0);
#endif
      }
    } else {
#pragma unroll
    for (int dz = 0; dz < KD; ++dz)
#pragma unroll
      for (int dy = 0; dy < KH; ++dy)
#pragma unroll
        for (int dx = 0; dx < KW; ++dx) {
          const int tap = (dz * KH + dy) * KW + dx;
          if (SPECIAL && TAPS == 27 && !((tapmask >> (tap & 31)) & 1u)) continue;
          if constexpr (NSUB > 0) {
            float a[NS1];
#pragma unroll
            for (int nn = 0; nn < NSUB; ++nn) a[nn] = Ww[tap * 4 * NTP + nn * 16];
#pragma unroll
            for (int m = 0; m < 4; ++m) {
              const float b = Xw[(dz * T::IY + (m * T::MR * T::RS + dy)) * T::IXS + dx];
#pragma unroll
              for (int nn = 0; nn < NSUB; ++nn)
                acc[m][nn] = __builtin_amdgcn_mfma_f32_16x16x4f32(a[nn], b, acc[m][nn], 0, 0, 0);
            }
          }
          if constexpr (REM > 0) {
            float xb[4];
#pragma unroll
            for (int cc = 0; cc < 4; ++cc) xb[cc] = Xr[cc * T::PLANEP + (dz * T::IY + dy) * T::IXS + dx];
#pragma unroll
            for (int q = 0; q < REM; ++q)
#pragma unroll
              for (int cc = 0; cc < 4; ++cc)
                accr[q] = __builtin_amdgcn_mfma_f32_4x4x1f32(Wr[(tap * 4 + cc) * NTP + 4 * q], xb[cc], accr[q], 0, 0, 0);
          }
        }
    }
  }

  const int oz = z0 + wv;
  constexpr bool stats_on = STATS;
  if (!stats_on && oz >= p.Do) return;
  if (stats_on) __syncthreads();
  auto emit = [&](int oy, int ox, int co, const f32x4& a4, float (&sa)[4], float (&sb)[4]) {
    if (oz >= p.Do || oy >= p.Ho || ox >= p.Wo || co >= p.Co) return;
    const int64_t v = (((int64_t)n * p.Do + oz) * p.Ho + oy) * p.Wo + ox;
    float4 r = make_float4(a4[0], a4[1], a4[2], a4[3]);
    if (gridDim.y > 1) {
      *reinterpret_cast<float4*>(partial + ((int64_t)blockIdx.y * p.N * p.Do * p.Ho * p.Wo + v) * p.Co + co) = r;
      return;
    }
    if (p.scale_mode) {
      const float4 s4 = *reinterpret_cast<const float4*>(scale + (p.scale_mode == 2 ? n * p.Co : 0) + co);
      r.x *= s4.x; r.y *= s4.y; r.z *= s4.z; r.w *= s4.w;
    }
    if (p.has_shift) {
      const float4 t = *reinterpret_cast<const float4*>(shift + co);
      r.x += t.x; r.y += t.y; r.z += t.z; r.w += t.w;
    }
    const int Cq = p.d2s_cq > 0 ? p.d2s_cq : CqP;
    const int q = p.d2s ? co / CqP : 0, oc = p.d2s ? co - q * CqP : co;
    if (p.d2s && oc >= Cq) return;
    if (p.res_mode) {
      int64_t rv = v;
      if (p.res_up2 && !p.d2s)
        rv = (((int64_t)n * (p.Do >> 1) + (oz >> 1)) * (p.Ho >> 1) + (oy >> 1)) * (p.Wo >> 1) + (ox >> 1);
      const float4 t = *reinterpret_cast<const float4*>(res + rv * (p.d2s ? Cq : p.Co) + oc);
      r.x += t.x; r.y += t.y; r.z += t.z; r.w += t.w;
    }
    r.x = cfun_apply_act(r.x, p.act, p.slope); r.y = cfun_apply_act(r.y, p.act, p.slope);
    r.z = cfun_apply_act(r.z, p.act, p.slope); r.w = cfun_apply_act(r.w, p.act, p.slope);
    if (stats_on) {
      sa[0] += r.x; sa[1] += r.y; sa[2] += r.z; sa[3] += r.w;
      sb[0] += r.x * r.x; sb[1] += r.y * r.y; sb[2] += r.z * r.z; sb[3] += r.w * r.w;
    }
    if (p.d2s) {
      const int64_t hv = (((int64_t)n * 2 * p.Do + 2 * oz + (q >> 2)) * 2 * p.Ho + 2 * oy + ((q >> 1) & 1)) * 2 * p.Wo +
                         2 * ox + (q & 1);
      *reinterpret_cast<float4*>(y + hv * Cq + oc) = r;
    } else {
      *reinterpret_cast<float4*>(y + v * p.Co + co) = r;
    }
  };
  constexpr int ES = stat_es(NT < STAT_ROUND ? NT : STAT_ROUND);
  const int tile = (int)(lid - (unsigned)n * per_n);
  if constexpr (NSUB > 0) {
#pragma unroll
    for (int nn = 0; nn < NSUB; ++nn) {
      float sa[4] = {0.f, 0.f, 0.f, 0.f}, sb[4] = {0.f, 0.f, 0.f, 0.f};
#pragma unroll
      for (int m = 0; m < 4; ++m) emit(y0 + m * T::MR + mrow, x0 + mx, cobase + nn * 16 + (lane >> 4) * 4, acc[m][nn], sa, sb);
      if constexpr (stats_on) {
        const int base = (nn * 16 / STAT_ROUND) * STAT_ROUND;
        quad_park_16(sa, sb, smem, ES, wv, lane, nn * 16 - base);
        const int end = (nn + 1) * 16;
        if (end % STAT_ROUND == 0 || end == NT) stat_round_flush(smem, ES, tid, base, end - base, cobase, n, tile, p, md);
      }
    }
  }
  if constexpr (REM > 0) {
    constexpr int RBASE = (16 * NSUB / STAT_ROUND) * STAT_ROUND;
    static_assert(16 * NSUB + 4 * REM - RBASE <= STAT_ROUND, "remainder quads must fit the last window");
#pragma unroll
    for (int q = 0; q < REM; ++q) {
      float sa[4] = {0.f, 0.f, 0.f, 0.f}, sb[4] = {0.f, 0.f, 0.f, 0.f};
      emit(y0 + lane / T::TW, x0 + lane % T::TW, cobase + 16 * NSUB + 4 * q, accr[q], sa, sb);
      if constexpr (stats_on) quad_park_wave(sa, sb, smem, ES, wv, lane, 16 * NSUB + 4 * q - RBASE);
    }
    if constexpr (stats_on) stat_round_flush(smem, ES, tid, RBASE, NT - RBASE, cobase, n, tile, p, md);
  }
}

inline int splitk_factor(int64_t nblk, int nchunks, const CfunConv3dParams& p, size_t ws_bytes) {
  if (p.d2s || nblk >= 768 || nchunks < 8) return 1;
  int k = nblk <= 128 ? (int)((512 + nblk - 1) / nblk) : (int)((1024 + nblk - 1) / nblk);
  if (k > nchunks / 4) k = nchunks / 4;
  if (k > 16) k = 16;
  const size_t per = (size_t)p.N * p.Do * p.Ho * p.Wo * p.Co * sizeof(float);
  while (k > 1 && (size_t)k * per > ws_bytes) --k;
  return k < 1 ? 1 : k;
}
inline size_t splitk_workspace(int64_t nblk, int nchunks, const CfunConv3dParams& p) {
  const int k = splitk_factor(nblk, nchunks, p, (size_t)-1);
  return k > 1 ? (size_t)k * p.N * p.Do * p.Ho * p.Wo * p.Co * sizeof(float) : 0;
}

template <int KD, int KH, int KW, int S, int NSUB, int REM = 0, int G = 0>
int launch_conv_mfma(const float* x, const float* wp, const float* scale, const float* shift, const float* res,
                     float* y, const CfunConv3dParams& p, const ConvMode& md, void* ws, size_t ws_bytes, hipStream_t st) {
  using T = FwdTile<KD, KH, KW, S, G>;
  constexpr int NT = 16 * NSUB + 4 * REM, NTP = row_stride(NT);
  if (REM > 0 && (p.Co % NT) != 0) return CFUN_EINVAL;
  const int ntz = cdiv(p.Do, T::TD), nty = cdiv(p.Ho, T::TH), ntx = cdiv(p.Wo, T::TW), ncot = cdiv(p.Co, NT);
  const int64_t nblk = (int64_t)p.N * ntz * nty * ntx * ncot;
  if (nblk == 0) return CFUN_OK;
  if (nblk > 0x7fffffffLL) return CFUN_EINVAL;
  constexpr bool kHasSpecial = (KD == 3 && KH == 3 && KW == 3 && S == 1);
  const bool special = md.in_s2d || md.tap_skip;
  if (special && !kHasSpecial) return CFUN_EINVAL;
  const bool upd = kHasSpecial && NSUB > 0 && REM == 0 && md.in_s2d && md.tap_skip == 2;
  const size_t lds = (size_t)(4 * T::PLANEP + ((md.tap_skip == 1 || upd) ? 8 : T::TAPS) * 4 * NTP) * sizeof(float);
  const int nchunks = md.in_s2d ? 8 * (md.in_cq >> 2) : (p.Ci >> 2);
  const int ksplit = splitk_factor(nblk, nchunks, p, ws_bytes);
  const bool stats = md.out_part != nullptr && ksplit == 1;
  auto kern = stats ? k_conv_mfma<KD, KH, KW, S, NSUB, 0, REM, true, G> : k_conv_mfma<KD, KH, KW, S, NSUB, 0, REM, false, G>;
  if constexpr (kHasSpecial) {
    if constexpr (G == 0) {
      if (special && md.tap_skip != 1)
        kern = stats ? k_conv_mfma<KD, KH, KW, S, NSUB, 1, REM, true> : k_conv_mfma<KD, KH, KW, S, NSUB, 1, REM, false>;
    } else {
      if (special && md.tap_skip != 1 && !upd) return CFUN_EINVAL;
    }
    if constexpr (NSUB > 0 && REM == 0) {
      if (md.tap_skip == 1) kern = stats ? k_conv_mfma<KD, KH, KW, S, NSUB, 2, 0, true, G> : k_conv_mfma<KD, KH, KW, S, NSUB, 2, 0, false, G>;
      if (upd) kern = k_conv_mfma<KD, KH, KW, S, NSUB, 3, 0, false, G>;
    } else {
      if (md.tap_skip == 1) return CFUN_EINVAL;
    }
  }
  size_t lds_k = lds;
  if (stats && lds_k < stat_lds_floats(NT) * sizeof(float)) lds_k = stat_lds_floats(NT) * sizeof(float);
  if (lds_k > 64 * 1024) {
    hipError_t e = hipFuncSetAttribute(reinterpret_cast<const void*>(kern), hipFuncAttributeMaxDynamicSharedMemorySize, (int)lds_k);
    if (e != hipSuccess) return (int)e;
  }
  const int cps = cdiv(nchunks, ksplit);
  ConvMode mk = md;
  mk.out_slots = ntz * nty * ntx * (p.d2s ? 8 : 1);
  if (ksplit > 1) mk.out_part = nullptr;
  hipLaunchKernelGGL(kern, dim3((unsigned)nblk, (unsigned)ksplit), dim3(256), lds_k, st, x, wp, scale, shift, res, y, p, mk,
                     ntz, nty, ntx, ncot, (float*)ws, cps);
  CFUN_LAUNCH_CHECK();
  if (ksplit > 1) return cfun_splitk_finish((const float*)ws, ksplit, scale, shift, res, y, &p, md.out_part, st);
  return CFUN_OK;
}

inline int tile_channels(int code) { return 16 * (code & 7) + 4 * (code >> 3); }

inline int fwd_stat_slots(int nsub, int geom, const CfunConv3dParams& p, const ConvMode& md, size_t ws_bytes) {
  const int nt = tile_channels(nsub);
  const int tiles = cdiv(p.Do, 4) * cdiv(p.Ho, geom ? 8 : 4) * cdiv(p.Wo, geom ? 8 : 16);
  const int64_t nblk = (int64_t)p.N * tiles * cdiv(p.Co, nt);
  const int nchunks = md.in_s2d ? 8 * (md.in_cq >> 2) : (p.Ci >> 2);
  return splitk_factor(nblk, nchunks, p, ws_bytes) > 1 ? -cfun_splitk_stat_slots(&p) : tiles * (p.d2s ? 8 : 1);
}

template <int KD, int KH, int KW, int S, int G = 0>
size_t fwd_workspace(int nsub, const CfunConv3dParams& p, const ConvMode& md) {
  using T = FwdTile<KD, KH, KW, S, G>;
  const int nt = tile_channels(nsub);
  const int64_t nblk = (int64_t)p.N * cdiv(p.Do, T::TD) * cdiv(p.Ho, T::TH) * cdiv(p.Wo, T::TW) * cdiv(p.Co, nt);
  const int nchunks = md.in_s2d ? 8 * (md.in_cq >> 2) : (p.Ci >> 2);
  return splitk_workspace(nblk, nchunks, p);
}

template <int KD, int KH, int KW, int S>
constexpr bool has_rem_tiles() {
  return (KD == 3 && KH == 3 && KW == 3) || (KD == 1 && KH == 1 && KW == 1 && S == 1);
}

template <int KD, int KH, int KW, int S>
constexpr int max_nsub() { return KD * KH * KW > 27 ? 1 : 5; }

template <int KD, int KH, int KW, int S, int G = 0>
int dispatch_nsub(int nsub, const float* x, const float* wp, const float* scale, const float* shift, const float* res,
                  float* y, const CfunConv3dParams& p, const ConvMode& flip, void* ws, size_t wsb, hipStream_t st) {
  if constexpr (has_rem_tiles<KD, KH, KW, S>()) {
    if (nsub == 1 + 8 * 1) return launch_conv_mfma<KD, KH, KW, S, 1, 1, G>(x, wp, scale, shift, res, y, p, flip, ws, wsb, st);
    if constexpr (G == 0)
      if (nsub == 2 + 8 * 2) return launch_conv_mfma<KD, KH, KW, S, 2, 2>(x, wp, scale, shift, res, y, p, flip, ws, wsb, st);
    if (nsub == 0 + 8 * 2) return launch_conv_mfma<KD, KH, KW, S, 0, 2, G>(x, wp, scale, shift, res, y, p, flip, ws, wsb, st);
  }
  if (nsub >= 8 || nsub < 1) return CFUN_EINVAL;
  if constexpr (max_nsub<KD, KH, KW, S>() == 1) {
    if (nsub != 1) return CFUN_EINVAL;
    return launch_conv_mfma<KD, KH, KW, S, 1, 0, G>(x, wp, scale, shift, res, y, p, flip, ws, wsb, st);
  } else {
    switch (nsub) {
      case 1: return launch_conv_mfma<KD, KH, KW, S, 1, 0, G>(x, wp, scale, shift, res, y, p, flip, ws, wsb, st);
      case 2: return launch_conv_mfma<KD, KH, KW, S, 2, 0, G>(x, wp, scale, shift, res, y, p, flip, ws, wsb, st);
      case 3: return launch_conv_mfma<KD, KH, KW, S, 3, 0, G>(x, wp, scale, shift, res, y, p, flip, ws, wsb, st);
      case 4: return launch_conv_mfma<KD, KH, KW, S, 4, 0, G>(x, wp, scale, shift, res, y, p, flip, ws, wsb, st);
      default: return launch_conv_mfma<KD, KH, KW, S, 5, 0, G>(x, wp, scale, shift, res, y, p, flip, ws, wsb, st);
    }
  }
}

struct WgIn {
  const float* stats;
  int act;
  float slope;
};

template <int KD, int KH, int KW, int S>
struct WgTile {
  static constexpr int TD = (S == 1) ? 2 : 1, TH = 4, TW = 16;
  static constexpr int TVOX = TD * TH * TW;
  static constexpr int TAPS = KD * KH * KW;
  static constexpr bool COMPACT = TAPS == 1;
  static constexpr int RS = COMPACT ? 1 : S;
  static constexpr int IZ = COMPACT ? TD : (TD - 1) * S + KD;
  static constexpr int IY = COMPACT ? TH : (TH - 1) * S + KH;
  static constexpr int IX = COMPACT ? TW : (TW - 1) * S + KW;
  static constexpr int IVOX = IZ * IY * IX;
  static constexpr int XS = 16;
  static constexpr int X_LOADS = cdiv(IVOX * 4, 256);
  static constexpr int TSPLIT = TAPS >= 4 ? 4 : 1;
  static constexpr int KSPLIT = 4 / TSPLIT;
  static constexpr int TPW = cdiv(TAPS, TSPLIT);
};

template <int KD, int KH, int KW, int S, int NSUB, bool TSKIP, int PACK, bool IN>
__device__ __forceinline__ void
wgrad_body(float* smem, const float* __restrict__ x, const float* __restrict__ g, float* __restrict__ partial,
           const CfunConv3dParams& p, int ntz, int nty, int ntx, int cot, int cis, int chunk, int tiles_per_chunk,
           int ntiles, const WgIn& fin) {
  using T = WgTile<KD, KH, KW, S>;
  constexpr int TAPS = T::TAPS, NT = 16 * NSUB, GS = pad_row16(NT);
  constexpr int NLIVE = TSKIP ? 8 : TAPS;
  constexpr int R = 16 / PACK;
  constexpr int TSPLIT = (TSKIP && NSUB <= 2) ? 1 : T::TSPLIT, KSPLIT = 4 / TSPLIT;
  constexpr int TPW = cdiv(cdiv(NLIVE, PACK), TSPLIT);
  constexpr int G_ITEMS = T::TVOX * (NT / 4);
  constexpr int G_LOADS = cdiv(G_ITEMS, 256);
  float* Xl = smem;
  float* Gl = smem + T::IVOX * T::XS;
  float4* Sl = reinterpret_cast<float4*>(Gl + T::TVOX * GS);

  const int tid = threadIdx.x, lane = tid & 63, wv = __builtin_amdgcn_readfirstlane(tid >> 6);
  const int ci0 = cis * 16;
  int cobase = cot * NT, colimit = NT, qpar = 0;
  if (TSKIP) {
    const int CqP = p.Co >> 3, tpp = cdiv(CqP, NT);
    qpar = cot / tpp;
    const int t = cot - qpar * tpp;
    cobase = qpar * CqP + t * NT;
    colimit = CqP - t * NT < NT ? CqP - t * NT : NT;
  }
  const int sh = p.up2 ? 1 : 0;
  const int Dv = p.Di << sh, Hv = p.Hi << sh, Wv = p.Wi << sh;
  const int tslot = wv % TSPLIT, kslot = wv / TSPLIT;

  f32x4 acc[TPW][NSUB];
#pragma unroll
  for (int t = 0; t < TPW; ++t)
#pragma unroll
    for (int nn = 0; nn < NSUB; ++nn) acc[t][nn] = f32x4{0.f, 0.f, 0.f, 0.f};

  float4 xin[T::X_LOADS], gin[G_LOADS];
  unsigned xvalid = 0, gvalid = 0;
  int n_table = -1;
  auto prefetch = [&](int tile) {
    int t = tile;
    const int tx = t % ntx; t /= ntx;
    const int ty = t % nty; t /= nty;
    const int tz = t % ntz;
    const int n = t / ntz;
    const int z0 = tz * T::TD, y0 = ty * T::TH, x0 = tx * T::TW;
    xvalid = 0; gvalid = 0;
    if constexpr (IN) {
      if (n != n_table) {
        n_table = n;
        if (tid < 8) {
          const int cs = ci0 + (tid >> 1) * 4;
          Sl[tid] = (fin.stats && cs < p.Ci) ? reinterpret_cast<const float4*>(fin.stats + ((int64_t)n * p.Ci + cs) * 2)[tid & 1]
                                             : make_float4(0.f, 1.f, 0.f, 1.f);
        }
      }
    }
#pragma unroll
    for (int i = 0; i < T::X_LOADS; ++i) {
      const int it = tid + i * 256;
      const int idx = it >> 2, c = ci0 + (it & 3) * 4;
      const int ix = idx % T::IX, iy = (idx / T::IX) % T::IY, iz = idx / (T::IX * T::IY);
      int vz, vy, vx;
      if (T::COMPACT) { vz = (z0 + iz) * S - p.pd; vy = (y0 + iy) * S - p.ph; vx = (x0 + ix) * S - p.pw; }
      else { vz = z0 * S - p.pd + iz; vy = y0 * S - p.ph + iy; vx = x0 * S - p.pw + ix; }
      const bool ok = (it < T::IVOX * 4) & (c < p.Ci) & (vz >= 0) & (vz < Dv) & (vy >= 0) & (vy < Hv) & (vx >= 0) &
                      (vx < Wv);
      const unsigned off = ((((unsigned)n * p.Di + (vz >> sh)) * p.Hi + (vy >> sh)) * p.Wi + (vx >> sh)) * p.Ci + c;
      xin[i] = *reinterpret_cast<const float4*>(x + (ok ? off : 0u));
      xvalid |= (ok ? 1u : 0u) << i;
    }
#pragma unroll
    for (int i = 0; i < G_LOADS; ++i) {
      const int it = tid + i * 256;
      const int vox = it / (NT / 4), col = (it % (NT / 4)) * 4;
      const int lx = vox % T::TW, ly = (vox / T::TW) % T::TH, lz = vox / (T::TW * T::TH);
      const int oz = z0 + lz, oy = y0 + ly, ox = x0 + lx;
      bool ok = (it < G_ITEMS) & (col < colimit) & (cobase + col < p.Co) & (oz < p.Do) & (oy < p.Ho) & (ox < p.Wo);
      unsigned off;
      if (p.d2s) {
        const int CqP = p.Co >> 3, Cq = p.d2s_cq > 0 ? p.d2s_cq : CqP;
        const int co = cobase + col, q = co / CqP, o = co - q * CqP;
        ok = ok & (o < Cq);
        off = ((((unsigned)n * 2 * p.Do + 2 * oz + (q >> 2)) * 2 * p.Ho + 2 * oy + ((q >> 1) & 1)) * 2 * p.Wo + 2 * ox +
               (q & 1)) * Cq + o;
      } else {
        off = ((((unsigned)n * p.Do + oz) * p.Ho + oy) * p.Wo + ox) * p.Co + cobase + col;
      }
      gin[i] = *reinterpret_cast<const float4*>(g + (ok ? off : 0u));
      gvalid |= (ok ? 1u : 0u) << i;
    }
  };
  auto commit = [&]() {
    auto keep = [](unsigned bit, const float4& v) {
      const float m = bit ? 1.f : 0.f;
      return make_float4(bit ? v.x : m, bit ? v.y : m, bit ? v.z : m, bit ? v.w : m);
    };
#pragma unroll
    for (int i = 0; i < T::X_LOADS; ++i) {
      const int it = tid + i * 256;
      if (it < T::IVOX * 4)
        *reinterpret_cast<float4*>(Xl + (it >> 2) * T::XS + (it & 3) * 4) =
            keep((xvalid >> i) & 1u, IN ? norm_act_in4(xin[i], Sl[(it & 3) * 2], Sl[(it & 3) * 2 + 1], fin.act, fin.slope) : xin[i]);
    }
#pragma unroll
    for (int i = 0; i < G_LOADS; ++i) {
      const int it = tid + i * 256;
      if (it < G_ITEMS)
        *reinterpret_cast<float4*>(Gl + (it / (NT / 4)) * GS + (it % (NT / 4)) * 4) = keep((gvalid >> i) & 1u, gin[i]);
    }
  };

  const int t_begin = chunk * tiles_per_chunk;
  const int t_end = (t_begin + tiles_per_chunk < ntiles) ? t_begin + tiles_per_chunk : ntiles;
  const float* Xw = Xl + (lane >> 4) * T::RS * T::XS + (PACK == 1 ? (lane & 15) : 0);
  const float* Gw = Gl + (lane >> 4) * GS + (lane & 15);

  auto live_tap = [&](int j, int& tap, int& off) {
    int dz, dy, dx;
    if (TSKIP) {
      dz = (qpar >> 2) + (j >> 2); dy = ((qpar >> 1) & 1) + ((j >> 1) & 1); dx = (qpar & 1) + (j & 1);
      tap = (dz * 3 + dy) * 3 + dx;
    } else {
      tap = j;
      dz = j / (KH * KW); dy = (j / KW) % KH; dx = j % KW;
    }
    off = ((dz * T::IY + dy) * T::IX + dx) * T::XS;
  };
  int toff[TPW];
#pragma unroll
  for (int t = 0; t < TPW; ++t) {
    int j = (t * TSPLIT + tslot) * PACK + (PACK == 1 ? 0 : (lane & 15) / R), tap;
    if (j >= NLIVE) j = NLIVE - 1;
    live_tap(j, tap, toff[t]);
    if (PACK > 1) toff[t] += (lane & 15) % R;
  }

  if (t_begin < t_end) prefetch(t_begin);
  for (int tile = t_begin; tile < t_end; ++tile) {
    __syncthreads();
    commit();
    __syncthreads();
    if (tile + 1 < t_end) prefetch(tile + 1);
#pragma unroll 4
    for (int it = 0; it < T::TVOX / 4 / KSPLIT; ++it) {
      const int grp = it * KSPLIT + kslot;
      const int xq = grp & 3, ly = (grp >> 2) & 3, lz = grp >> 4;
      float b[NSUB], a[TPW];
#pragma unroll
      for (int nn = 0; nn < NSUB; ++nn) b[nn] = Gw[(grp * 4) * GS + nn * 16];
      const float* Xg = Xw + ((lz * T::RS * T::IY + ly * T::RS) * T::IX + xq * 4 * T::RS) * T::XS;
#pragma unroll
      for (int t = 0; t < TPW; ++t) a[t] = Xg[toff[t]];
#pragma unroll
      for (int t = 0; t < TPW; ++t)
#pragma unroll
        for (int nn = 0; nn < NSUB; ++nn)
          acc[t][nn] = __builtin_amdgcn_mfma_f32_16x16x4f32(a[t], b[nn], acc[t][nn], 0, 0, 0);
    }
  }

  float* out = partial + (int64_t)(chunk * KSPLIT + kslot) * TAPS * p.Ci * p.CoP;
#pragma unroll
  for (int t = 0; t < TPW; ++t) {
#pragma unroll
    for (int r = 0; r < 4; ++r) {
      const int i = (lane >> 4) * 4 + r;
      const int j = (t * TSPLIT + tslot) * PACK + i / R, ci = ci0 + i % R;
      if (j >= NLIVE || ci >= p.Ci) continue;
      int tap, off;
      live_tap(j, tap, off);
#pragma unroll
      for (int nn = 0; nn < NSUB; ++nn) {
        const int co = cobase + nn * 16 + (lane & 15);
        if (co < p.CoP && nn * 16 + (lane & 15) < colimit) out[((int64_t)tap * p.Ci + ci) * p.CoP + co] = acc[t][nn][r];
      }
    }
  }
  if (TSKIP) {
    const unsigned live = parity_tapmask(qpar, false);
    for (int tap = 0; tap < TAPS; ++tap) {
      if ((live >> tap) & 1u) continue;
      for (int e = (KSPLIT == 1 ? tid : lane); e < 16 * NT; e += (KSPLIT == 1 ? 256 : 64)) {
        const int ci = ci0 + e / NT, col = e % NT, co = cobase + col;
        if (ci < p.Ci && col < colimit && co < p.CoP) out[((int64_t)tap * p.Ci + ci) * p.CoP + co] = 0.f;
      }
    }
  }
}

template <int KD, int KH, int KW, int S, int NSUB, bool TSKIP, int PACK, bool IN = false>
__global__ void __launch_bounds__(256)
k_wgrad_mfma(const float* __restrict__ x, const float* __restrict__ g, float* __restrict__ partial,
             CfunConv3dParams p, int ntz, int nty, int ntx, int ncisub, int ncot, int tiles_per_chunk, int ntiles, WgIn fin) {
  CFUN_DYN_LDS(float, smem);
  unsigned lid = xcd_remap(blockIdx.x, gridDim.x);
  const int cot = lid % ncot; lid /= ncot;
  const int cis = lid % ncisub;
  const int chunk = lid / ncisub;
  wgrad_body<KD, KH, KW, S, NSUB, TSKIP, PACK, IN>(smem, x, g, partial, p, ntz, nty, ntx, cot, cis, chunk,
                                                   tiles_per_chunk, ntiles, fin);
}

template <int KD, int KH, int KW, int S>
constexpr bool wgrad_fused_shape() { return KD * KH * KW == 27; }

inline int wgrad_fused_mode(const CfunConv3dParams& p, int nsub) {
  if (p.kd * p.kh * p.kw != 27 || (p.d2s && p.tap_skip) || nsub > 3) return 0;
  if (p.Ci > 16 && p.Ci <= 20) return 1 | (4 << 4);
  if (p.Ci > 32 && p.Ci <= 40 && p.stride == 1) return 2 | (2 << 4);
  return 0;
}

template <int KD, int KH, int KW, int S, int NSUB, int NPL, int PACK, bool IN = false>
__global__ void __launch_bounds__(256)
k_wgrad_fused(const float* __restrict__ x, const float* __restrict__ g, float* __restrict__ partial, CfunConv3dParams p,
              int ntz, int nty, int ntx, int ncot, int tiles_per_chunk, int ntiles, WgIn fin) {
  using T = WgTile<KD, KH, KW, S>;
  constexpr int TAPS = T::TAPS, NT = 16 * NSUB, GS = pad_row16(NT);
  constexpr int R = 16 / PACK, CH = 16 * NPL + R, C4 = CH / 4;
  constexpr int XS = CH == 20 ? 24 : CH;
  constexpr int TPW = cdiv(TAPS, 4);
  constexpr int NQ = cdiv(TAPS, PACK);
  constexpr int TPP = cdiv(NQ, 4);
  constexpr int X_ITEMS = T::IVOX * C4, X_LOADS = cdiv(X_ITEMS, 256);
  constexpr int G_ITEMS = T::TVOX * (NT / 4), G_LOADS = cdiv(G_ITEMS, 256);
  CFUN_DYN_LDS(float, smem);
  float* Xl = smem;
  float* Gl = smem + T::IVOX * XS;
  float4* Sl = reinterpret_cast<float4*>(Gl + T::TVOX * GS);

  const int tid = threadIdx.x, lane = tid & 63, wv = __builtin_amdgcn_readfirstlane(tid >> 6);
  unsigned lid = xcd_remap(blockIdx.x, gridDim.x);
  const int cot = lid % ncot;
  const int chunk = lid / ncot;
  const int cobase = cot * NT;
  const int sh = p.up2 ? 1 : 0;
  const int Dv = p.Di << sh, Hv = p.Hi << sh, Wv = p.Wi << sh;

  f32x4 acc[NPL][TPW][NSUB], accp[TPP][NSUB];
#pragma unroll
  for (int nn = 0; nn < NSUB; ++nn) {
#pragma unroll
    for (int s = 0; s < NPL; ++s)
#pragma unroll
      for (int t = 0; t < TPW; ++t) acc[s][t][nn] = f32x4{0.f, 0.f, 0.f, 0.f};
#pragma unroll
    for (int u = 0; u < TPP; ++u) accp[u][nn] = f32x4{0.f, 0.f, 0.f, 0.f};
  }

  float4 xin[X_LOADS], gin[G_LOADS];
  unsigned xvalid = 0, gvalid = 0;
  int n_table = -1;
  auto prefetch = [&](int tile) {
    int t = tile;
    const int tx = t % ntx; t /= ntx;
    const int ty = t % nty; t /= nty;
    const int tz = t % ntz;
    const int n = t / ntz;
    if constexpr (IN) {
      if (n != n_table) {
        n_table = n;
        if (tid < 2 * C4) {
          const int cs = (tid >> 1) * 4;
          Sl[tid] = (fin.stats && cs < p.Ci) ? reinterpret_cast<const float4*>(fin.stats + ((int64_t)n * p.Ci + cs) * 2)[tid & 1]
                                             : make_float4(0.f, 1.f, 0.f, 1.f);
        }
      }
    }
    const int z0 = tz * T::TD, y0 = ty * T::TH, x0 = tx * T::TW;
    xvalid = 0; gvalid = 0;
#pragma unroll
    for (int i = 0; i < X_LOADS; ++i) {
      const int it = tid + i * 256;
      const int idx = it / C4, c = (it - idx * C4) * 4;
      const int ix = idx % T::IX, iy = (idx / T::IX) % T::IY, iz = idx / (T::IX * T::IY);
      const int vz = z0 * S - p.pd + iz, vy = y0 * S - p.ph + iy, vx = x0 * S - p.pw + ix;
      const bool ok = (it < X_ITEMS) & (c < p.Ci) & (vz >= 0) & (vz < Dv) & (vy >= 0) & (vy < Hv) & (vx >= 0) & (vx < Wv);
      const unsigned off = ((((unsigned)n * p.Di + (vz >> sh)) * p.Hi + (vy >> sh)) * p.Wi + (vx >> sh)) * p.Ci + c;
      xin[i] = *reinterpret_cast<const float4*>(x + (ok ? off : 0u));
      xvalid |= (ok ? 1u : 0u) << i;
    }
#pragma unroll
    for (int i = 0; i < G_LOADS; ++i) {
      const int it = tid + i * 256;
      const int vox = it / (NT / 4), col = (it % (NT / 4)) * 4;
      const int lx = vox % T::TW, ly = (vox / T::TW) % T::TH, lz = vox / (T::TW * T::TH);
      const int oz = z0 + lz, oy = y0 + ly, ox = x0 + lx;
      bool ok = (it < G_ITEMS) & (cobase + col < p.Co) & (oz < p.Do) & (oy < p.Ho) & (ox < p.Wo);
      unsigned off;
      if (p.d2s) {
        const int CqP = p.Co >> 3, Cq = p.d2s_cq > 0 ? p.d2s_cq : CqP;
        const int co = cobase + col, q = co / CqP, o = co - q * CqP;
        ok = ok & (o < Cq);
        off = ((((unsigned)n * 2 * p.Do + 2 * oz + (q >> 2)) * 2 * p.Ho + 2 * oy + ((q >> 1) & 1)) * 2 * p.Wo + 2 * ox +
               (q & 1)) * Cq + o;
      } else {
        off = ((((unsigned)n * p.Do + oz) * p.Ho + oy) * p.Wo + ox) * p.Co + cobase + col;
      }
      gin[i] = *reinterpret_cast<const float4*>(g + (ok ? off : 0u));
      gvalid |= (ok ? 1u : 0u) << i;
    }
  };
  auto commit = [&]() {
    auto keep = [](unsigned bit, const float4& v) {
      const float m = bit ? 1.f : 0.f;
      return make_float4(bit ? v.x : m, bit ? v.y : m, bit ? v.z : m, bit ? v.w : m);
    };
#pragma unroll
    for (int i = 0; i < X_LOADS; ++i) {
      const int it = tid + i * 256;
      if (it < X_ITEMS) {
        const int idx = it / C4, c = (it - idx * C4) * 4;
        *reinterpret_cast<float4*>(Xl + idx * XS + c) =
            keep((xvalid >> i) & 1u, IN ? norm_act_in4(xin[i], Sl[(c >> 2) * 2], Sl[(c >> 2) * 2 + 1], fin.act, fin.slope) : xin[i]);
      }
    }
#pragma unroll
    for (int i = 0; i < G_LOADS; ++i) {
      const int it = tid + i * 256;
      if (it < G_ITEMS)
        *reinterpret_cast<float4*>(Gl + (it / (NT / 4)) * GS + (it % (NT / 4)) * 4) = keep((gvalid >> i) & 1u, gin[i]);
    }
  };

  const int t_begin = chunk * tiles_per_chunk;
  const int t_end = (t_begin + tiles_per_chunk < ntiles) ? t_begin + tiles_per_chunk : ntiles;
  const float* Xv = Xl + (lane >> 4) * T::RS * XS;
  const float* Gw = Gl + (lane >> 4) * GS + (lane & 15);
  auto tap_off = [&](int tap) {
    const int dz = tap / (KH * KW), dy = (tap / KW) % KH, dx = tap % KW;
    return ((dz * T::IY + dy) * T::IX + dx) * XS;
  };
  int toff[TPW], toffp[TPP];
#pragma unroll
  for (int t = 0; t < TPW; ++t) {
    const int tap = t * 4 + wv;
    toff[t] = tap_off(tap < TAPS ? tap : TAPS - 1) + (lane & 15);
  }
#pragma unroll
  for (int u = 0; u < TPP; ++u) {
    const int tap = (u * 4 + wv) * PACK + (lane & 15) / R;
    toffp[u] = tap_off(tap < TAPS ? tap : TAPS - 1) + 16 * NPL + (lane & 15) % R;
  }

  if (t_begin < t_end) prefetch(t_begin);
  for (int tile = t_begin; tile < t_end; ++tile) {
    __syncthreads();
    commit();
    __syncthreads();
    if (tile + 1 < t_end) prefetch(tile + 1);
#pragma unroll 2
    for (int grp = 0; grp < T::TVOX / 4; ++grp) {
      const int xq = grp & 3, ly = (grp >> 2) & 3, lz = grp >> 4;
      float b[NSUB], a[NPL][TPW], ap[TPP];
#pragma unroll
      for (int nn = 0; nn < NSUB; ++nn) b[nn] = Gw[(grp * 4) * GS + nn * 16];
      const float* Xg = Xv + ((lz * T::RS * T::IY + ly * T::RS) * T::IX + xq * 4 * T::RS) * XS;
#pragma unroll
      for (int s = 0; s < NPL; ++s)
#pragma unroll
        for (int t = 0; t < TPW; ++t) a[s][t] = Xg[toff[t] + 16 * s];
#pragma unroll
      for (int u = 0; u < TPP; ++u) ap[u] = Xg[toffp[u]];
#pragma unroll
      for (int s = 0; s < NPL; ++s)
#pragma unroll
        for (int t = 0; t < TPW; ++t)
#pragma unroll
          for (int nn = 0; nn < NSUB; ++nn)
            acc[s][t][nn] = __builtin_amdgcn_mfma_f32_16x16x4f32(a[s][t], b[nn], acc[s][t][nn], 0, 0, 0);
#pragma unroll
      for (int u = 0; u < TPP; ++u)
#pragma unroll
        for (int nn = 0; nn < NSUB; ++nn)
          accp[u][nn] = __builtin_amdgcn_mfma_f32_16x16x4f32(ap[u], b[nn], accp[u][nn], 0, 0, 0);
    }
  }

  float* out = partial + (int64_t)chunk * TAPS * p.Ci * p.CoP;
#pragma unroll
  for (int nn = 0; nn < NSUB; ++nn) {
    const int co = cobase + nn * 16 + (lane & 15);
    if (co >= p.CoP) continue;
#pragma unroll
    for (int r = 0; r < 4; ++r) {
      const int i = (lane >> 4) * 4 + r;
#pragma unroll
      for (int t = 0; t < TPW; ++t) {
        const int tap = t * 4 + wv;
        if (tap < TAPS) {
#pragma unroll
          for (int s = 0; s < NPL; ++s) out[((int64_t)tap * p.Ci + 16 * s + i) * p.CoP + co] = acc[s][t][nn][r];
        }
      }
#pragma unroll
      for (int u = 0; u < TPP; ++u) {
        const int tap = (u * 4 + wv) * PACK + i / R, ci = 16 * NPL + i % R;
        if (tap < TAPS && ci < p.Ci) out[((int64_t)tap * p.Ci + ci) * p.CoP + co] = accp[u][nn][r];
      }
    }
  }
}

struct WgPlan {
  int ntz, nty, ntx, ntiles, ncisub, ncot, nchunks, tiles_per_chunk, nsub, kslots;
  const float* in_stats;
  int in_act;
  float in_slope;
};


template <int KD, int KH, int KW, int S>
WgPlan wgrad_plan(const CfunConv3dParams& p, int nsub) {
  using T = WgTile<KD, KH, KW, S>;
  WgPlan w;
  w.nsub = nsub;
  w.ntz = cdiv(p.Do, T::TD); w.nty = cdiv(p.Ho, T::TH); w.ntx = cdiv(p.Wo, T::TW);
  w.ntiles = p.N * w.ntz * w.nty * w.ntx;
  w.ncisub = (wgrad_fused_shape<KD, KH, KW, S>() && wgrad_fused_mode(p, nsub)) ? 1 : cdiv(p.Ci, 16);
  w.ncot = (p.d2s && p.tap_skip) ? 8 * cdiv(p.Co >> 3, 16 * nsub) : cdiv(p.CoP, 16 * nsub);
  int want = 512 / (w.ncisub * w.ncot);
  if (want < 1) want = 1;
  if (want > w.ntiles) want = w.ntiles;
  if (want < 1) want = 1;
  w.tiles_per_chunk = cdiv(w.ntiles, want);
  if (w.tiles_per_chunk < 1) w.tiles_per_chunk = 1;
  w.nchunks = cdiv(w.ntiles, w.tiles_per_chunk);
  if (w.nchunks < 1) w.nchunks = 1;
  w.kslots = (p.d2s && p.tap_skip && T::TAPS == 27 && nsub <= 2) ? 4 : T::KSPLIT;
  w.in_stats = nullptr; w.in_act = 0; w.in_slope = 0.f;
  return w;
}

template <int KD, int KH, int KW, int S, int NSUB>
int launch_wgrad_mfma(const float* x, const float* g, float* partial, const CfunConv3dParams& p, const WgPlan& w,
                      hipStream_t st) {
  using T = WgTile<KD, KH, KW, S>;
  constexpr int NT = 16 * NSUB, GS = pad_row16(NT);
  const size_t lds = (size_t)(T::IVOX * T::XS + T::TVOX * GS) * sizeof(float) + 8 * sizeof(float4);
  const int64_t lim = (int64_t)1 << 31;
  if ((int64_t)p.N * p.Di * p.Hi * p.Wi * p.Ci >= lim || (int64_t)p.N * p.Do * p.Ho * p.Wo * p.Co >= lim) return CFUN_EINVAL;
  if constexpr (wgrad_fused_shape<KD, KH, KW, S>() && NSUB <= 3) {
    const int mode = wgrad_fused_mode(p, NSUB);
    if (mode) {
      const int xs = (mode & 15) == 1 ? 24 : 40;
      const size_t ldsf = (size_t)(T::IVOX * xs + T::TVOX * GS) * sizeof(float) + 2 * (xs / 4) * sizeof(float4);
      const bool in = w.in_stats != nullptr || w.in_act != CFUN_ACT_NONE;
      void (*kf)(const float*, const float*, float*, CfunConv3dParams, int, int, int, int, int, int, WgIn) =
          in ? k_wgrad_fused<KD, KH, KW, S, NSUB, 1, 4, true> : k_wgrad_fused<KD, KH, KW, S, NSUB, 1, 4, false>;
      if constexpr (S == 1) {
        if ((mode & 15) == 2) kf = in ? k_wgrad_fused<KD, KH, KW, S, NSUB, 2, 2, true> : k_wgrad_fused<KD, KH, KW, S, NSUB, 2, 2, false>;
      }
      if (ldsf > 64 * 1024) {
        hipError_t e = hipFuncSetAttribute(reinterpret_cast<const void*>(kf), hipFuncAttributeMaxDynamicSharedMemorySize, (int)ldsf);
        if (e != hipSuccess) return (int)e;
      }
      hipLaunchKernelGGL(kf, dim3((unsigned)(w.nchunks * w.ncot)), dim3(256), ldsf, st, x, g, partial, p, w.ntz, w.nty,
                         w.ntx, w.ncot, w.tiles_per_chunk, w.ntiles, WgIn{w.in_stats, w.in_act, w.in_slope});
      CFUN_LAUNCH_CHECK();
      return CFUN_OK;
    }
  }
  const bool in = w.in_stats != nullptr || w.in_act != CFUN_ACT_NONE;
  auto kern = k_wgrad_mfma<KD, KH, KW, S, NSUB, false, 1, false>;
  auto pick = [&](auto in_c) {
    constexpr bool I = decltype(in_c)::value;
    kern = k_wgrad_mfma<KD, KH, KW, S, NSUB, false, 1, I>;
    if constexpr (KD * KH * KW == 27) {
      const int pack = w.ncisub > 1 ? 1 : p.Ci <= 4 ? 4 : p.Ci <= 8 ? 2 : 1;
      const bool ts = S == 1 && p.d2s && p.tap_skip;
      if constexpr (S == 1) {
        if (ts) kern = pack == 4 ? k_wgrad_mfma<KD, KH, KW, S, NSUB, true, 4, I>
                     : pack == 2 ? k_wgrad_mfma<KD, KH, KW, S, NSUB, true, 2, I>
                                 : k_wgrad_mfma<KD, KH, KW, S, NSUB, true, 1, I>;
      }
      if (!ts) kern = pack == 4 ? k_wgrad_mfma<KD, KH, KW, S, NSUB, false, 4, I>
                    : pack == 2 ? k_wgrad_mfma<KD, KH, KW, S, NSUB, false, 2, I>
                                : k_wgrad_mfma<KD, KH, KW, S, NSUB, false, 1, I>;
    }
  };
  if (in) pick(std::true_type{}); else pick(std::false_type{});
  if (lds > 64 * 1024) {
    hipError_t e = hipFuncSetAttribute(reinterpret_cast<const void*>(kern), hipFuncAttributeMaxDynamicSharedMemorySize, (int)lds);
    if (e != hipSuccess) return (int)e;
  }
  const int64_t nblk = (int64_t)w.nchunks * w.ncisub * w.ncot;
  hipLaunchKernelGGL(kern, dim3((unsigned)nblk), dim3(256), lds, st, x, g, partial, p, w.ntz, w.nty, w.ntx, w.ncisub,
                     w.ncot, w.tiles_per_chunk, w.ntiles, WgIn{w.in_stats, w.in_act, w.in_slope});
  CFUN_LAUNCH_CHECK();
  return CFUN_OK;
}

template <int KD, int KH, int KW, int S>
int dispatch_wgrad(const float* x, const float* g, float* partial, const CfunConv3dParams& p, const WgPlan& w,
                   hipStream_t st) {
  if constexpr (max_nsub<KD, KH, KW, S>() == 1) {
    if (w.nsub != 1) return CFUN_EINVAL;
    return launch_wgrad_mfma<KD, KH, KW, S, 1>(x, g, partial, p, w, st);
  } else {
    switch (w.nsub) {
      case 1: return launch_wgrad_mfma<KD, KH, KW, S, 1>(x, g, partial, p, w, st);
      case 2: return launch_wgrad_mfma<KD, KH, KW, S, 2>(x, g, partial, p, w, st);
      case 3: return launch_wgrad_mfma<KD, KH, KW, S, 3>(x, g, partial, p, w, st);
      case 4: return launch_wgrad_mfma<KD, KH, KW, S, 4>(x, g, partial, p, w, st);
      default: return launch_wgrad_mfma<KD, KH, KW, S, 5>(x, g, partial, p, w, st);
    }
  }
}

}

#define CFUN_MFMA_DECL(NAME)                                                                                        \
  int cfun_mfma_fwd_##NAME(int nsub, const float* x, const float* wp, const float* scale, const float* shift,       \
                           const float* res, float* y, const CfunConv3dParams& p, const cfun_mfma::ConvMode& flip,  \
                           void* ws, size_t wsb, hipStream_t st);                                                   \
  size_t cfun_mfma_fwd_ws_##NAME(int nsub, const CfunConv3dParams& p, const cfun_mfma::ConvMode& md);               \
  void cfun_mfma_wgrad_plan_##NAME(const CfunConv3dParams& p, int nsub, cfun_mfma::WgPlan* w);                      \
  int cfun_mfma_wgrad_##NAME(const float* x, const float* g, float* partial, const CfunConv3dParams& p,             \
                             const cfun_mfma::WgPlan& w, hipStream_t st);

#define CFUN_MFMA_DEFINE(NAME, KD, KH, KW, S)                                                                       \
  int cfun_mfma_fwd_##NAME(int nsub, const float* x, const float* wp, const float* scale, const float* shift,       \
                           const float* res, float* y, const CfunConv3dParams& p, const cfun_mfma::ConvMode& flip,  \
                           void* ws, size_t wsb, hipStream_t st) {                                                  \
    return cfun_mfma::dispatch_nsub<KD, KH, KW, S>(nsub, x, wp, scale, shift, res, y, p, flip, ws, wsb, st);        \
  }                                                                                                                 \
  size_t cfun_mfma_fwd_ws_##NAME(int nsub, const CfunConv3dParams& p, const cfun_mfma::ConvMode& md) {              \
    return cfun_mfma::fwd_workspace<KD, KH, KW, S>(nsub, p, md);                                                    \
  }                                                                                                                 \
  void cfun_mfma_wgrad_plan_##NAME(const CfunConv3dParams& p, int nsub, cfun_mfma::WgPlan* w) {                     \
    *w = cfun_mfma::wgrad_plan<KD, KH, KW, S>(p, nsub);                                                             \
  }                                                                                                                 \
  int cfun_mfma_wgrad_##NAME(const float* x, const float* g, float* partial, const CfunConv3dParams& p,             \
                             const cfun_mfma::WgPlan& w, hipStream_t st) {                                          \
    return cfun_mfma::dispatch_wgrad<KD, KH, KW, S>(x, g, partial, p, w, st);                                       \
  }

#define CFUN_MFMA_DECL_G8(NAME)                                                                                     \
  int cfun_mfma_fwd_g8_##NAME(int nsub, const float* x, const float* wp, const float* scale, const float* shift,    \
                              const float* res, float* y, const CfunConv3dParams& p,                                \
                              const cfun_mfma::ConvMode& flip, void* ws, size_t wsb, hipStream_t st);               \
  size_t cfun_mfma_fwd_ws_g8_##NAME(int nsub, const CfunConv3dParams& p, const cfun_mfma::ConvMode& md);

#define CFUN_MFMA_DEFINE_G8(NAME, KD, KH, KW, S)                                                                    \
  int cfun_mfma_fwd_g8_##NAME(int nsub, const float* x, const float* wp, const float* scale, const float* shift,    \
                              const float* res, float* y, const CfunConv3dParams& p,                                \
                              const cfun_mfma::ConvMode& flip, void* ws, size_t wsb, hipStream_t st) {              \
    return cfun_mfma::dispatch_nsub<KD, KH, KW, S, 1>(nsub, x, wp, scale, shift, res, y, p, flip, ws, wsb, st);     \
  }                                                                                                                 \
  size_t cfun_mfma_fwd_ws_g8_##NAME(int nsub, const CfunConv3dParams& p, const cfun_mfma::ConvMode& md) {           \
    return cfun_mfma::fwd_workspace<KD, KH, KW, S, 1>(nsub, p, md);                                                 \
  }

CFUN_MFMA_DECL_G8(k333s1)
CFUN_MFMA_DECL_G8(k333s2)
CFUN_MFMA_DECL_G8(k222s1)

int cfun_tile_geom(const CfunConv3dParams* p, int g8_exists);

CFUN_MFMA_DECL(k333s1)
CFUN_MFMA_DECL(k333s2)
CFUN_MFMA_DECL(k111s1)
CFUN_MFMA_DECL(k111s2)
CFUN_MFMA_DECL(k133s1)
CFUN_MFMA_DECL(k311s1)
CFUN_MFMA_DECL(k555s1)
CFUN_MFMA_DECL(k222s1)
```

cfun_amd/csrc/conv3d_wino_wgrad.hip:

```cpp
#include <stdlib.h>

#include "conv3d_mfma.h"

int cfun_wino_shape_ok(const CfunConv3dParams* p);

namespace {

using cfun_mfma::cdiv;

constexpr int WG_IY = 6, WG_XH = 9, WG_XROWS = 4 * WG_IY;
constexpr int WG_XVOX = WG_XROWS * 2 * WG_XH;
constexpr int WG_GVOX = 2 * 4 * 16;
constexpr int WG_XROW = 2 * WG_XH * 16;

template <int NSUB, bool D2S>
__global__ void __launch_bounds__(256)
k_wgrad_wino(const float* __restrict__ x, const float* __restrict__ g, float* __restrict__ partial, CfunConv3dParams p,
             int ntz, int nty, int ntx, int ncisub, int ncot, int tiles_per_chunk, int ntiles) {
  constexpr int NT = 16 * NSUB, GS = cfun_mfma::pad_row16(NT);
  constexpr int X_ITEMS = WG_XVOX * 4, X_LOADS = cdiv(X_ITEMS, 256);
  constexpr int G_ITEMS = WG_GVOX * (NT / 4), G_LOADS = cdiv(G_ITEMS, 256);
  CFUN_DYN_LDS(float4, smem4);
  float* Xl = reinterpret_cast<float*>(smem4);
  float* Gl = Xl + WG_XVOX * 16;

  const int tid = threadIdx.x, lane = tid & 63, wv = __builtin_amdgcn_readfirstlane(tid >> 6);
  unsigned lid = cfun_mfma::xcd_remap(blockIdx.x, gridDim.x);
  const int cot = lid % ncot; lid /= ncot;
  const int cis = lid % ncisub;
  const int chunk = lid / ncisub;
  const int ci0 = cis * 16, cobase = cot * NT;

  f32x4 acc[9][NSUB];
#pragma unroll
  for (int r = 0; r < 9; ++r)
#pragma unroll
    for (int nn = 0; nn < NSUB; ++nn) acc[r][nn] = f32x4{0.f, 0.f, 0.f, 0.f};

  float4 xin[X_LOADS], gin[G_LOADS];
  unsigned xvalid = 0, gvalid = 0;
  auto prefetch = [&](int tile) {
    int t = tile;
    const int tx = t % ntx; t /= ntx;
    const int ty = t % nty; t /= nty;
    const int tz = t % ntz;
    const int n = t / ntz;
    const int z0 = tz * 2, y0 = ty * 4, x0 = tx * 16;
    xvalid = 0; gvalid = 0;
#pragma unroll
    for (int i = 0; i < X_LOADS; ++i) {
      const int it = tid + i * 256;
      const int idx = it >> 2, c = ci0 + (it & 3) * 4;
      const int xh = idx % WG_XH, par = (idx / WG_XH) & 1, row = idx / (2 * WG_XH);
      const int vz = z0 - p.pd + row / WG_IY, vy = y0 - 1 + row % WG_IY, vx = x0 - 1 + 2 * xh + par;
      const bool ok = (it < X_ITEMS) & (c < p.Ci) & (vz >= 0) & (vz < p.Di) & (vy >= 0) & (vy < p.Hi) & (vx >= 0) & (vx < p.Wi);
      const unsigned off = ((((unsigned)n * p.Di + vz) * p.Hi + vy) * p.Wi + vx) * p.Ci + c;
      xin[i] = *reinterpret_cast<const float4*>(x + (ok ? off : 0u));
      xvalid |= (ok ? 1u : 0u) << i;
    }
#pragma unroll
    for (int i = 0; i < G_LOADS; ++i) {
      const int it = tid + i * 256;
      const int slot = it / (NT / 4), col = (it % (NT / 4)) * 4;
      const int j = slot & 7, par = (slot >> 3) & 1, lrow = slot >> 4;
      const int oz = z0 + (lrow >> 2), oy = y0 + (lrow & 3), ox = x0 + 2 * j + par;
      bool ok = (it < G_ITEMS) & (cobase + col < p.Co) & (oz < p.Do) & (oy < p.Ho) & (ox < p.Wo);
      unsigned off;
      if (D2S) {
        const int CqP = p.Co >> 3, Cq = p.d2s_cq > 0 ? p.d2s_cq : CqP;
        const int co = cobase + col, q = co / CqP, o = co - q * CqP;
        ok = ok & (o < Cq);
        off = ((((unsigned)n * 2 * p.Do + 2 * oz + (q >> 2)) * 2 * p.Ho + 2 * oy + ((q >> 1) & 1)) * 2 * p.Wo + 2 * ox +
               (q & 1)) * Cq + o;
      } else {
        off = ((((unsigned)n * p.Do + oz) * p.Ho + oy) * p.Wo + ox) * p.Co + cobase + col;
      }
      gin[i] = *reinterpret_cast<const float4*>(g + (ok ? off : 0u));
      gvalid |= (ok ? 1u : 0u) << i;
    }
  };
  auto commit = [&]() {
    auto keep = [](unsigned bit, const float4& v) {
      const float m = bit ? 1.f : 0.f;
      return make_float4(bit ? v.x : m, bit ? v.y : m, bit ? v.z : m, bit ? v.w : m);
    };
#pragma unroll
    for (int i = 0; i < X_LOADS; ++i) {
      const int it = tid + i * 256;
      if (it < X_ITEMS) *reinterpret_cast<float4*>(Xl + it * 4) = keep((xvalid >> i) & 1u, xin[i]);
    }
#pragma unroll
    for (int i = 0; i < G_LOADS; ++i) {
      const int it = tid + i * 256;
      if (it < G_ITEMS)
        *reinterpret_cast<float4*>(Gl + (it / (NT / 4)) * GS + (it % (NT / 4)) * 4) = keep((gvalid >> i) & 1u, gin[i]);
    }
  };

  const int o1 = wv == 0 ? 0 : wv == 2 ? 16 : WG_XH * 16;
  const int o2 = wv == 2 ? WG_XH * 16 : wv == 3 ? WG_XH * 16 + 16 : 16;
  const float s2 = wv == 1 ? 1.f : -1.f;
  const float ce = wv == 3 ? 0.f : 1.f, cg = wv == 0 ? 0.f : wv == 1 ? 1.f : -1.f;
  const float* Xa1 = Xl + o1 + (lane >> 4) * 16 + (lane & 15);
  const float* Xa2 = Xl + o2 + (lane >> 4) * 16 + (lane & 15);
  const float* Gw = Gl + (lane >> 4) * GS + (lane & 15);

  const int t_begin = chunk * tiles_per_chunk;
  const int t_end = (t_begin + tiles_per_chunk < ntiles) ? t_begin + tiles_per_chunk : ntiles;
  if (t_begin < t_end) prefetch(t_begin);
  for (int tile = t_begin; tile < t_end; ++tile) {
    __syncthreads();
    commit();
    __syncthreads();
    if (tile + 1 < t_end) prefetch(tile + 1);
#pragma unroll 1
    for (int grp = 0; grp < 16; ++grp) {
      const int lrow = grp >> 1, q = grp & 1;
      const int hrow = (lrow >> 2) * WG_IY + (lrow & 3);
      float b[NSUB], a[9];
#pragma unroll
      for (int nn = 0; nn < NSUB; ++nn) {
        const float* gp = Gw + ((lrow * 2) * 8 + q * 4) * GS + nn * 16;
        b[nn] = ce * gp[0] + cg * gp[8 * GS];
      }
      const float* x1 = Xa1 + hrow * WG_XROW + q * 64;
      const float* x2 = Xa2 + hrow * WG_XROW + q * 64;
#pragma unroll
      for (int r = 0; r < 9; ++r) {
        const int o = ((r / 3) * WG_IY + (r % 3)) * WG_XROW;
        a[r] = x1[o] + s2 * x2[o];
      }
#pragma unroll
      for (int r = 0; r < 9; ++r)
#pragma unroll
        for (int nn = 0; nn < NSUB; ++nn)
          acc[r][nn] = __builtin_amdgcn_mfma_f32_16x16x4f32(a[r], b[nn], acc[r][nn], 0, 0, 0);
    }
  }

  float* S = Xl;
  float* out = partial + (int64_t)chunk * 27 * p.Ci * p.CoP;
#pragma unroll
  for (int r9 = 0; r9 < 9; ++r9) {
    __syncthreads();
#pragma unroll
    for (int nn = 0; nn < NSUB; ++nn)
#pragma unroll
      for (int r = 0; r < 4; ++r)
        S[(wv * 16 + (lane >> 4) * 4 + r) * NT + nn * 16 + (lane & 15)] = acc[r9][nn][r];
    __syncthreads();
    for (int e = tid; e < 16 * NT; e += 256) {
      const int ci = ci0 + e / NT, co = cobase + e % NT;
      if (ci >= p.Ci || co >= p.CoP) continue;
      const float u0 = S[e], u1 = S[16 * NT + e], u2 = S[2 * 16 * NT + e], u3 = S[3 * 16 * NT + e];
      const float h = 0.5f * (u1 + u2);
      float* o = out + ((int64_t)(r9 * 3) * p.Ci + ci) * p.CoP + co;
      o[0] = u0 + h;
      o[(int64_t)p.Ci * p.CoP] = 0.5f * (u1 - u2);
      o[2 * (int64_t)p.Ci * p.CoP] = u3 + h;
    }
  }
}

template <int NSUB, bool D2S>
__global__ void __launch_bounds__(512)
k_wgrad_wino2(const float* __restrict__ x, const float* __restrict__ g, float* __restrict__ partial, CfunConv3dParams p,
              int ntz, int nty, int ntx, int ncisub, int ncot, int tiles_per_chunk, int ntiles) {
  constexpr int NT = 16 * NSUB, GS = cfun_mfma::pad_row16(NT);
  constexpr int X_ITEMS = WG_XVOX * 4, X_LOADS = cdiv(X_ITEMS, 512);
  constexpr int G_ITEMS = WG_GVOX * (NT / 4), G_LOADS = cdiv(G_ITEMS, 512);
  CFUN_DYN_LDS(float4, smem4);
  float* Xl = reinterpret_cast<float*>(smem4);
  float* Gl = Xl + WG_XVOX * 16;

  const int tid = threadIdx.x, lane = tid & 63, wv = __builtin_amdgcn_readfirstlane(tid >> 6);
  unsigned lid = cfun_mfma::xcd_remap(blockIdx.x, gridDim.x);
  const int cot = lid % ncot; lid /= ncot;
  const int cis = lid % ncisub;
  const int chunk = lid / ncisub;
  const int ci0 = cis * 16, cobase = cot * NT;

  f32x4 acc[3][2][NSUB];
#pragma unroll
  for (int dz = 0; dz < 3; ++dz)
#pragma unroll
    for (int h = 0; h < 2; ++h)
#pragma unroll
      for (int nn = 0; nn < NSUB; ++nn) acc[dz][h][nn] = f32x4{0.f, 0.f, 0.f, 0.f};

  float4 xin[X_LOADS], gin[G_LOADS];
  unsigned xvalid = 0, gvalid = 0;
  auto prefetch = [&](int tile) {
    int t = tile;
    const int tx = t % ntx; t /= ntx;
    const int ty = t % nty; t /= nty;
    const int tz = t % ntz;
    const int n = t / ntz;
    const int z0 = tz * 2, y0 = ty * 4, x0 = tx * 16;
    xvalid = 0; gvalid = 0;
#pragma unroll
    for (int i = 0; i < X_LOADS; ++i) {
      const int it = tid + i * 512;
      const int idx = it >> 2, c = ci0 + (it & 3) * 4;
      const int xh = idx % WG_XH, par = (idx / WG_XH) & 1, row = idx / (2 * WG_XH);
      const int vz = z0 - p.pd + row / WG_IY, vy = y0 - 1 + row % WG_IY, vx = x0 - 1 + 2 * xh + par;
      const bool ok = (it < X_ITEMS) & (c < p.Ci) & (vz >= 0) & (vz < p.Di) & (vy >= 0) & (vy < p.Hi) & (vx >= 0) & (vx < p.Wi);
      const unsigned off = ((((unsigned)n * p.Di + vz) * p.Hi + vy) * p.Wi + vx) * p.Ci + c;
      xin[i] = *reinterpret_cast<const float4*>(x + (ok ? off : 0u));
      xvalid |= (ok ? 1u : 0u) << i;
    }
#pragma unroll
    for (int i = 0; i < G_LOADS; ++i) {
      const int it = tid + i * 512;
      const int slot = it / (NT / 4), col = (it % (NT / 4)) * 4;
      const int j = slot & 7, par = (slot >> 3) & 1, lrow = slot >> 4;
      const int oz = z0 + (lrow >> 2), oy = y0 + (lrow & 3), ox = x0 + 2 * j + par;
      bool ok = (it < G_ITEMS) & (cobase + col < p.Co) & (oz < p.Do) & (oy < p.Ho) & (ox < p.Wo);
      unsigned off;
      if (D2S) {
        const int CqP = p.Co >> 3, Cq = p.d2s_cq > 0 ? p.d2s_cq : CqP;
        const int co = cobase + col, q = co / CqP, o = co - q * CqP;
        ok = ok & (o < Cq);
        off = ((((unsigned)n * 2 * p.Do + 2 * oz + (q >> 2)) * 2 * p.Ho + 2 * oy + ((q >> 1) & 1)) * 2 * p.Wo + 2 * ox +
               (q & 1)) * Cq + o;
      } else {
        off = ((((unsigned)n * p.Do + oz) * p.Ho + oy) * p.Wo + ox) * p.Co + cobase + col;
      }
      gin[i] = *reinterpret_cast<const float4*>(g + (ok ? off : 0u));
      gvalid |= (ok ? 1u : 0u) << i;
    }
  };
  auto commit = [&]() {
    auto keep = [](unsigned bit, const float4& v) {
      const float m = bit ? 1.f : 0.f;
      return make_float4(bit ? v.x : m, bit ? v.y : m, bit ? v.z : m, bit ? v.w : m);
    };
#pragma unroll
    for (int i = 0; i < X_LOADS; ++i) {
      const int it = tid + i * 512;
      if (it < X_ITEMS) *reinterpret_cast<float4*>(Xl + it * 4) = keep((xvalid >> i) & 1u, xin[i]);
    }
#pragma unroll
    for (int i = 0; i < G_LOADS; ++i) {
      const int it = tid + i * 512;
      if (it < G_ITEMS)
        *reinterpret_cast<float4*>(Gl + (it / (NT / 4)) * GS + (it % (NT / 4)) * 4) = keep((gvalid >> i) & 1u, gin[i]);
    }
  };

  const int py = wv >> 1, h = wv & 1;
  const int rA = py == 0 ? 0 : py == 2 ? 2 : 1, rB = py == 0 ? 2 : py == 1 ? 2 : py == 2 ? 1 : 3;
  const float sy = py == 1 ? 1.f : -1.f;
  const int cofs0 = h ? 144 : 0, cofs1 = h ? 16 : 144, cofs2 = h ? 160 : 16;
  const float lo0 = h ? -1.f : 1.f, lo1 = h ? 1.f : 0.f, lo2 = h ? 0.f : -1.f;
  const float hi0 = h ? 1.f : 0.f, hi1 = h ? 0.f : 1.f, hi2 = h ? -1.f : 1.f;
  const float ye = py == 3 ? 0.f : 1.f, yo = py == 0 ? 0.f : py == 1 ? 1.f : -1.f;
  const float xle = 1.f, xlo = h ? -1.f : 0.f;
  const float xhe = h ? 0.f : 1.f, xho = h ? -1.f : 1.f;
  const float* Xw = Xl + (lane >> 4) * 16 + (lane & 15);
  const float* Gw = Gl + (lane >> 4) * GS + (lane & 15);

  const int t_begin = chunk * tiles_per_chunk;
  const int t_end = (t_begin + tiles_per_chunk < ntiles) ? t_begin + tiles_per_chunk : ntiles;
  if (t_begin < t_end) prefetch(t_begin);
  for (int tile = t_begin; tile < t_end; ++tile) {
    __syncthreads();
    commit();
    __syncthreads();
    if (tile + 1 < t_end) prefetch(tile + 1);
#pragma unroll 1
    for (int ks = 0; ks < 8; ++ks) {
      const int lz = ks >> 2, yp = (ks >> 1) & 1, q = ks & 1;
      float b[2][NSUB];
#pragma unroll
      for (int nn = 0; nn < NSUB; ++nn) {
        const float* gp = Gw + (((lz * 4 + 2 * yp) * 2) * 8 + q * 4) * GS + nn * 16;
        const float te = ye * gp[0] + yo * gp[2 * 8 * GS];
        const float to = ye * gp[8 * GS] + yo * gp[3 * 8 * GS];
        b[0][nn] = xle * te + xlo * to;
        b[1][nn] = xhe * te + xho * to;
      }
      const float* xq = Xw + ((lz * WG_IY + 2 * yp) * WG_XROW) + q * 64;
#pragma unroll
      for (int dz = 0; dz < 3; ++dz) {
        const float* xa = xq + (dz * WG_IY + rA) * WG_XROW;
        const float* xb = xq + (dz * WG_IY + rB) * WG_XROW;
        const float a0 = xa[cofs0], a1 = xa[cofs1], a2 = xa[cofs2];
        const float b0 = xb[cofs0], b1 = xb[cofs1], b2 = xb[cofs2];
        const float vlo = (lo0 * a0 + (lo1 * a1 + lo2 * a2)) + sy * (lo0 * b0 + (lo1 * b1 + lo2 * b2));
        const float vhi = (hi0 * a0 + (hi1 * a1 + hi2 * a2)) + sy * (hi0 * b0 + (hi1 * b1 + hi2 * b2));
#pragma unroll
        for (int nn = 0; nn < NSUB; ++nn) {
          acc[dz][0][nn] = __builtin_amdgcn_mfma_f32_16x16x4f32(vlo, b[0][nn], acc[dz][0][nn], 0, 0, 0);
          acc[dz][1][nn] = __builtin_amdgcn_mfma_f32_16x16x4f32(vhi, b[1][nn], acc[dz][1][nn], 0, 0, 0);
        }
      }
    }
  }

  float* S = Xl;
  float* out = partial + (int64_t)chunk * 27 * p.Ci * p.CoP;
#pragma unroll
  for (int dz = 0; dz < 3; ++dz) {
    __syncthreads();
#pragma unroll
    for (int hh = 0; hh < 2; ++hh)
#pragma unroll
      for (int nn = 0; nn < NSUB; ++nn)
#pragma unroll
        for (int r = 0; r < 4; ++r)
          S[((py * 4 + 2 * h + hh) * 16 + (lane >> 4) * 4 + r) * NT + nn * 16 + (lane & 15)] = acc[dz][hh][nn][r];
    __syncthreads();
    for (int e = tid; e < 16 * NT; e += 512) {
      const int ci = ci0 + e / NT, co = cobase + e % NT;
      if (ci >= p.Ci || co >= p.CoP) continue;
      float t[3][4];
#pragma unroll
      for (int px = 0; px < 4; ++px) {
        const float u0 = S[(0 * 4 + px) * 16 * NT + e], u1 = S[(1 * 4 + px) * 16 * NT + e], u2 = S[(2 * 4 + px) * 16 * NT + e],
                    u3 = S[(3 * 4 + px) * 16 * NT + e];
        const float hsum = 0.5f * (u1 + u2);
        t[0][px] = u0 + hsum; t[1][px] = 0.5f * (u1 - u2); t[2][px] = u3 + hsum;
      }
#pragma unroll
      for (int ky = 0; ky < 3; ++ky) {
        const float hsum = 0.5f * (t[ky][1] + t[ky][2]);
        float* o = out + ((int64_t)((dz * 3 + ky) * 3) * p.Ci + ci) * p.CoP + co;
        o[0] = t[ky][0] + hsum;
        o[(int64_t)p.Ci * p.CoP] = 0.5f * (t[ky][1] - t[ky][2]);
        o[2 * (int64_t)p.Ci * p.CoP] = t[ky][3] + hsum;
      }
    }
  }
}

struct WgPlanW {
  int nsub, ntz, nty, ntx, ntiles, ncisub, ncot, nchunks, tiles_per_chunk;
};

WgPlanW make_wg_plan(const CfunConv3dParams& p) {
  WgPlanW w;
  w.nsub = p.CoP <= 16 ? 1 : ((p.CoP + 31) / 32 * 32 < (p.CoP + 47) / 48 * 48 ? 2 : 3);
  w.ntz = cdiv(p.Do, 2); w.nty = cdiv(p.Ho, 4); w.ntx = cdiv(p.Wo, 16);
  w.ntiles = p.N * w.ntz * w.nty * w.ntx;
  w.ncisub = cdiv(p.Ci, 16);
  w.ncot = cdiv(p.CoP, 16 * w.nsub);
  static int knob = -1;
  if (knob < 0) {
    const char* e = getenv("CFUN_WINO_WGRAD_WGS");
    knob = e && atoi(e) > 0 ? atoi(e) : 0;
  }
  const int pairs = w.ncisub * w.ncot;
  const int total = knob ? knob : pairs >= 100 ? 1024 : pairs >= 48 ? 768 : 512;
  int want = total / pairs;
  if (want > w.ntiles) want = w.ntiles;
  if (want < 1) want = 1;
  w.tiles_per_chunk = cdiv(w.ntiles, want);
  if (w.tiles_per_chunk < 1) w.tiles_per_chunk = 1;
  w.nchunks = cdiv(w.ntiles, w.tiles_per_chunk);
  if (w.nchunks < 1) w.nchunks = 1;
  return w;
}

int wino_wgrad_2d(const CfunConv3dParams& p) {
  static int knob = -2;
  if (knob == -2) {
    const char* e = getenv("CFUN_WINO_WGRAD_2D");
    knob = e ? atoi(e) : -1;
  }
  if (CFUN_ALGO_OF(p.algo) == CFUN_ALGO_WINO) return 0;
  if (CFUN_ALGO_OF(p.algo) == CFUN_ALGO_WINO2 || knob == 1) return 1;
  return 0;
}

template <int NSUB>
int launch_wg2(const float* x, const float* g, float* partial, const CfunConv3dParams& p, const WgPlanW& w, hipStream_t st) {
  constexpr int GS = cfun_mfma::pad_row16(16 * NSUB);
  size_t lds = (size_t)(WG_XVOX * 16 + WG_GVOX * GS) * sizeof(float);
  const size_t scratch = (size_t)16 * 16 * 16 * NSUB * sizeof(float);
  if (lds < scratch) lds = scratch;
  auto kern = p.d2s ? k_wgrad_wino2<NSUB, true> : k_wgrad_wino2<NSUB, false>;
  if (lds > 64 * 1024) {
    hipError_t e = hipFuncSetAttribute(reinterpret_cast<const void*>(kern), hipFuncAttributeMaxDynamicSharedMemorySize, (int)lds);
    if (e != hipSuccess) return (int)e;
  }
  hipLaunchKernelGGL(kern, dim3((unsigned)(w.nchunks * w.ncisub * w.ncot)), dim3(512), lds, st, x, g, partial, p, w.ntz,
                     w.nty, w.ntx, w.ncisub, w.ncot, w.tiles_per_chunk, w.ntiles);
  CFUN_LAUNCH_CHECK();
  return CFUN_OK;
}

template <int NSUB>
int launch_wg(const float* x, const float* g, float* partial, const CfunConv3dParams& p, const WgPlanW& w, hipStream_t st) {
  constexpr int GS = cfun_mfma::pad_row16(16 * NSUB);
  size_t lds = (size_t)(WG_XVOX * 16 + WG_GVOX * GS) * sizeof(float);
  const size_t scratch = (size_t)4 * 16 * 16 * NSUB * sizeof(float);
  if (lds < scratch) lds = scratch;
  auto kern = p.d2s ? k_wgrad_wino<NSUB, true> : k_wgrad_wino<NSUB, false>;
  if (lds > 64 * 1024) {
    hipError_t e = hipFuncSetAttribute(reinterpret_cast<const void*>(kern), hipFuncAttributeMaxDynamicSharedMemorySize, (int)lds);
    if (e != hipSuccess) return (int)e;
  }
  hipLaunchKernelGGL(kern, dim3((unsigned)(w.nchunks * w.ncisub * w.ncot)), dim3(256), lds, st, x, g, partial, p, w.ntz,
                     w.nty, w.ntx, w.ncisub, w.ncot, w.tiles_per_chunk, w.ntiles);
  CFUN_LAUNCH_CHECK();
  return CFUN_OK;
}

}

int cfun_wino_wgrad_supported(const CfunConv3dParams* p) {
  static int knob = -2;
  if (knob == -2) {
    const char* e = getenv("CFUN_WINO_WGRAD");
    knob = e ? atoi(e) : -1;
  }
  if (knob == 0 || !cfun_wino_shape_ok(p)) return 0;
  const int64_t lim = (int64_t)1 << 31;
  if ((int64_t)p->N * p->Di * p->Hi * p->Wi * p->Ci >= lim || (int64_t)p->N * p->Do * p->Ho * p->Wo * p->Co >= lim) return 0;
  if (knob == 1 || CFUN_ALGO_OF(p->algo) == CFUN_ALGO_WINO || CFUN_ALGO_OF(p->algo) == CFUN_ALGO_WINO2) return 1;
  if (p->d2s) return 0;
  return !(p->Ci <= 8 || (p->Ci > 16 && p->Ci <= 20));
}

size_t cfun_wino_wgrad_workspace_bytes(const CfunConv3dParams* p) {
  const WgPlanW w = make_wg_plan(*p);
  return (size_t)w.nchunks * 27 * p->Ci * p->CoP * sizeof(float);
}

int cfun_wino_wgrad(const float* x, const float* g, float* ws, const CfunConv3dParams* p, int* nparts, hipStream_t st) {
  const WgPlanW w = make_wg_plan(*p);
  *nparts = w.nchunks;
  if (wino_wgrad_2d(*p)) {
    switch (w.nsub) {
      case 1: return launch_wg2<1>(x, g, ws, *p, w, st);
      case 2: return launch_wg2<2>(x, g, ws, *p, w, st);
      default: return launch_wg2<3>(x, g, ws, *p, w, st);
    }
  }
  switch (w.nsub) {
    case 1: return launch_wg<1>(x, g, ws, *p, w, st);
    case 2: return launch_wg<2>(x, g, ws, *p, w, st);
    default: return launch_wg<3>(x, g, ws, *p, w, st);
  }
}
```

include/cfun_tile.h:

```cpp
#ifndef CFUN_TILE_H
#define CFUN_TILE_H

#include "cfun_hip.h"

#ifdef __cplusplus
extern "C" {
#endif

int cfun_conv3d_fwd_tile(const CfunConv3dParams* p, int32_t out[3]);

#ifdef __cplusplus
}
#endif

#endif
```

Baseline: 25.93 volumes/s.

## Add 8x8 spatial tile geometry for MFMA and Winograd weight-gradient kernels

Adds a second tile geometry (TH=8, TW=8 instead of 4x16) to the MFMA and Winograd wgrad kernels, templated on G. Selection goes through cfun_tile_geom with heuristics that skip the 8x8 geometry where it would lose a wave. The aim is better halo reuse and fewer wasted edge voxels on volumes whose width is not a multiple of 16. It also sets an occupancy hint in launch bounds for one Winograd variant and exports a query for the chosen wgrad tile. In exchange it adds many template instantiations and risks register or LDS pressure changes.

```diff
diff --git a/cfun_amd/_lib.py b/cfun_amd/_lib.py
--- a/cfun_amd/_lib.py
+++ b/cfun_amd/_lib.py
@@ -148,6 +148,7 @@
 
 TILE_SIGNATURES = {
     "cfun_conv3d_fwd_tile": (C.c_int, [_PP, C.POINTER(C.c_int32)]),
+    "cfun_conv3d_wgrad_tile": (C.c_int, [_PP, C.POINTER(C.c_int32)]),
 }
 TILE_EXPORTS = tuple(TILE_SIGNATURES)
 
diff --git a/cfun_amd/csrc/conv3d.hip b/cfun_amd/csrc/conv3d.hip
--- a/cfun_amd/csrc/conv3d.hip
+++ b/cfun_amd/csrc/conv3d.hip
@@ -28,6 +28,7 @@
 int cfun_wino_wgrad_supported(const CfunConv3dParams*);
 size_t cfun_wino_wgrad_workspace_bytes(const CfunConv3dParams*);
 int cfun_wino_wgrad(const float*, const float*, float*, const CfunConv3dParams*, int*, hipStream_t);
+int cfun_wino_wgrad_geom(const CfunConv3dParams*);
 int cfun_wgrad_c1_supported(const CfunConv3dParams*);
 size_t cfun_wgrad_c1_ws(const CfunConv3dParams*);
 int cfun_wgrad_c1(const float*, const float*, CfunWgradDst, const CfunConv3dParams*, void*, size_t, hipStream_t);
@@ -49,18 +50,24 @@
   int max_nsub;
   FwdFn fwd8;
   FwdWsFn fwd_ws8;
+  PlanFn plan8;
+  WgFn wgrad8;
 };
 
-#define SHAPE(NAME, KD, KH, KW, S, MAXN) \
-  { KD, KH, KW, S, cfun_mfma_fwd_##NAME, cfun_mfma_fwd_ws_##NAME, cfun_mfma_wgrad_plan_##NAME, cfun_mfma_wgrad_##NAME, MAXN, \
-    nullptr, nullptr }
-#define SHAPE_G8(NAME, KD, KH, KW, S, MAXN) \
-  { KD, KH, KW, S, cfun_mfma_fwd_##NAME, cfun_mfma_fwd_ws_##NAME, cfun_mfma_wgrad_plan_##NAME, cfun_mfma_wgrad_##NAME, MAXN, \
-    cfun_mfma_fwd_g8_##NAME, cfun_mfma_fwd_ws_g8_##NAME }
+#define SHAPE_BASE(NAME, KD, KH, KW, S, MAXN) \
+  KD, KH, KW, S, cfun_mfma_fwd_##NAME, cfun_mfma_fwd_ws_##NAME, cfun_mfma_wgrad_plan_##NAME, cfun_mfma_wgrad_##NAME, MAXN
+#define FWD_G8(NAME) cfun_mfma_fwd_g8_##NAME, cfun_mfma_fwd_ws_g8_##NAME
+#define WGRAD_G8(NAME) cfun_mfma_wgrad_plan_g8_##NAME, cfun_mfma_wgrad_g8_##NAME
+#define NO_G8 nullptr, nullptr
 const Shape kShapes[] = {
-    SHAPE_G8(k333s1, 3, 3, 3, 1, 5), SHAPE_G8(k333s2, 3, 3, 3, 2, 5), SHAPE(k111s1, 1, 1, 1, 1, 5),
-    SHAPE(k111s2, 1, 1, 1, 2, 5), SHAPE(k133s1, 1, 3, 3, 1, 5), SHAPE(k311s1, 3, 1, 1, 1, 5),
-    SHAPE(k555s1, 5, 5, 5, 1, 1), SHAPE_G8(k222s1, 2, 2, 2, 1, 5),
+    {SHAPE_BASE(k333s1, 3, 3, 3, 1, 5), FWD_G8(k333s1), WGRAD_G8(k333s1)},
+    {SHAPE_BASE(k333s2, 3, 3, 3, 2, 5), FWD_G8(k333s2), WGRAD_G8(k333s2)},
+    {SHAPE_BASE(k111s1, 1, 1, 1, 1, 5), NO_G8, WGRAD_G8(k111s1)},
+    {SHAPE_BASE(k111s2, 1, 1, 1, 2, 5), NO_G8, NO_G8},
+    {SHAPE_BASE(k133s1, 1, 3, 3, 1, 5), NO_G8, NO_G8},
+    {SHAPE_BASE(k311s1, 3, 1, 1, 1, 5), NO_G8, NO_G8},
+    {SHAPE_BASE(k555s1, 5, 5, 5, 1, 1), NO_G8, NO_G8},
+    {SHAPE_BASE(k222s1, 2, 2, 2, 1, 5), FWD_G8(k222s1), NO_G8},
 };
 
 const Shape* find_shape(int kd, int kh, int kw, int s) {
@@ -660,6 +667,15 @@
   return (int64_t)p->N * p->Di * p->Hi * p->Wi * p->Ci < lim && go < lim;
 }
 
+static bool wgrad_g8_loses_wave(const CfunConv3dParams* p, const Shape* s, int nsub) {
+  if (s->kd != 3 || s->s != 1) return false;
+  return (p->d2s && p->tap_skip && nsub == 5) || (p->Ci <= 4 && nsub == 4);
+}
+
+static int wgrad_geom(const CfunConv3dParams* p, const Shape* s) {
+  return cfun_tile_geom(p, !s->wgrad8 ? 0 : wgrad_g8_loses_wave(p, s, wgrad_nsub(p, s)) ? 2 : 1);
+}
+
 size_t cfun_conv3d_bwd_weight_workspace_bytes(const CfunConv3dParams* p) {
   if (!valid_params(p)) return 0;
   if (CFUN_ALGO_OF(p->algo) != CFUN_ALGO_DIRECT && cfun_wgrad_c1_supported(p)) return cfun_align_up(cfun_wgrad_c1_ws(p), 256);
@@ -667,7 +683,7 @@
   if (s && cfun_wino_wgrad_supported(p)) return cfun_align_up(cfun_wino_wgrad_workspace_bytes(p), 256);
   if (s) {
     cfun_mfma::WgPlan w;
-    s->plan(*p, wgrad_nsub(p, s), &w);
+    (wgrad_geom(p, s) ? s->plan8 : s->plan)(*p, wgrad_nsub(p, s), &w);
     return cfun_align_up((size_t)w.nchunks * w.kslots * p->kd * p->kh * p->kw * p->Ci * p->CoP * sizeof(float), 256);
   }
   return cfun_align_up(cfun_direct_wgrad_ws(p), 256);
@@ -699,18 +715,29 @@
       return cfun_wgrad_finish((const float*)ws, dst, p, nparts, cfun_st(stream));
     }
     cfun_mfma::WgPlan w;
-    s->plan(*p, wgrad_nsub(p, s), &w);
+    const int geom = wgrad_geom(p, s);
+    (geom ? s->plan8 : s->plan)(*p, wgrad_nsub(p, s), &w);
     if (pro) {
       if (f->in_act != CFUN_ACT_NONE && (f->in_act != CFUN_ACT_LRELU || f->in_slope < 0.f || f->in_slope > 1.f)) return CFUN_EINVAL;
       w.in_stats = f->in_stats; w.in_act = CFUN_ACT_LRELU; w.in_slope = f->in_act == CFUN_ACT_LRELU ? f->in_slope : 1.f;
     }
     if (w.ntiles == 0) return cfun_wgrad_zero(dst, p, cfun_st(stream));
-    const int rc = s->wgrad(x, g, (float*)ws, *p, w, cfun_st(stream));
+    const int rc = (geom ? s->wgrad8 : s->wgrad)(x, g, (float*)ws, *p, w, cfun_st(stream));
     if (rc) return rc;
     return cfun_wgrad_finish((const float*)ws, dst, p, w.nchunks * w.kslots, cfun_st(stream));
   }
   if (CFUN_ALGO_OF(p->algo) == CFUN_ALGO_MFMA) return CFUN_EINVAL;
   return cfun_conv_bwd_weight_direct(x, g, dst, p, ws, ws_bytes, cfun_st(stream));
+}
+
+int cfun_conv3d_wgrad_tile(const CfunConv3dParams* p, int32_t out[3]) {
+  if (!out || !valid_params(p)) return CFUN_EINVAL;
+  if (CFUN_ALGO_OF(p->algo) == CFUN_ALGO_DIRECT || cfun_wgrad_c1_supported(p) || !wgrad_mfma_fits(p)) return CFUN_EINVAL;
+  const Shape* s = mfma_shape(p);
+  if (!s) return CFUN_EINVAL;
+  const int g = cfun_wino_wgrad_supported(p) ? cfun_wino_wgrad_geom(p) : wgrad_geom(p, s);
+  out[0] = p->stride == 1 ? 2 : 1; out[1] = g ? 8 : 4; out[2] = g ? 8 : 16;
+  return CFUN_OK;
 }
 
 int cfun_conv3d_bwd_weight(const float* x, const float* g, float* dwp, const CfunConv3dParams* p, void* ws,
diff --git a/cfun_amd/csrc/conv3d_mfma.h b/cfun_amd/csrc/conv3d_mfma.h
--- a/cfun_amd/csrc/conv3d_mfma.h
+++ b/cfun_amd/csrc/conv3d_mfma.h
@@ -554,9 +554,10 @@
   float slope;
 };
 
-template <int KD, int KH, int KW, int S>
+template <int KD, int KH, int KW, int S, int G = 0>
 struct WgTile {
-  static constexpr int TD = (S == 1) ? 2 : 1, TH = 4, TW = 16;
+  static constexpr int TD = (S == 1) ? 2 : 1, TH = G ? 8 : 4, TW = G ? 8 : 16;
+  static constexpr int XQ = TW / 4;
   static constexpr int TVOX = TD * TH * TW;
   static constexpr int TAPS = KD * KH * KW;
   static constexpr bool COMPACT = TAPS == 1;
@@ -572,12 +573,12 @@
   static constexpr int TPW = cdiv(TAPS, TSPLIT);
 };
 
-template <int KD, int KH, int KW, int S, int NSUB, bool TSKIP, int PACK, bool IN>
+template <int KD, int KH, int KW, int S, int NSUB, bool TSKIP, int PACK, bool IN, int G>
 __device__ __forceinline__ void
 wgrad_body(float* smem, const float* __restrict__ x, const float* __restrict__ g, float* __restrict__ partial,
            const CfunConv3dParams& p, int ntz, int nty, int ntx, int cot, int cis, int chunk, int tiles_per_chunk,
            int ntiles, const WgIn& fin) {
-  using T = WgTile<KD, KH, KW, S>;
+  using T = WgTile<KD, KH, KW, S, G>;
   constexpr int TAPS = T::TAPS, NT = 16 * NSUB, GS = pad_row16(NT);
   constexpr int NLIVE = TSKIP ? 8 : TAPS;
   constexpr int R = 16 / PACK;
@@ -719,7 +720,7 @@
 #pragma unroll 4
     for (int it = 0; it < T::TVOX / 4 / KSPLIT; ++it) {
       const int grp = it * KSPLIT + kslot;
-      const int xq = grp & 3, ly = (grp >> 2) & 3, lz = grp >> 4;
+      const int xq = grp % T::XQ, ly = (grp / T::XQ) % T::TH, lz = grp / (T::XQ * T::TH);
       float b[NSUB], a[TPW];
 #pragma unroll
       for (int nn = 0; nn < NSUB; ++nn) b[nn] = Gw[(grp * 4) * GS + nn * 16];
@@ -763,7 +764,7 @@
   }
 }
 
-template <int KD, int KH, int KW, int S, int NSUB, bool TSKIP, int PACK, bool IN = false>
+template <int KD, int KH, int KW, int S, int NSUB, bool TSKIP, int PACK, bool IN = false, int G = 0>
 __global__ void __launch_bounds__(256)
 k_wgrad_mfma(const float* __restrict__ x, const float* __restrict__ g, float* __restrict__ partial,
              CfunConv3dParams p, int ntz, int nty, int ntx, int ncisub, int ncot, int tiles_per_chunk, int ntiles, WgIn fin) {
@@ -772,8 +773,8 @@
   const int cot = lid % ncot; lid /= ncot;
   const int cis = lid % ncisub;
   const int chunk = lid / ncisub;
-  wgrad_body<KD, KH, KW, S, NSUB, TSKIP, PACK, IN>(smem, x, g, partial, p, ntz, nty, ntx, cot, cis, chunk,
-                                                   tiles_per_chunk, ntiles, fin);
+  wgrad_body<KD, KH, KW, S, NSUB, TSKIP, PACK, IN, G>(smem, x, g, partial, p, ntz, nty, ntx, cot, cis, chunk,
+                                                      tiles_per_chunk, ntiles, fin);
 }
 
 template <int KD, int KH, int KW, int S>
@@ -786,11 +787,11 @@
   return 0;
 }
 
-template <int KD, int KH, int KW, int S, int NSUB, int NPL, int PACK, bool IN = false>
+template <int KD, int KH, int KW, int S, int NSUB, int NPL, int PACK, bool IN = false, int G = 0>
 __global__ void __launch_bounds__(256)
 k_wgrad_fused(const float* __restrict__ x, const float* __restrict__ g, float* __restrict__ partial, CfunConv3dParams p,
               int ntz, int nty, int ntx, int ncot, int tiles_per_chunk, int ntiles, WgIn fin) {
-  using T = WgTile<KD, KH, KW, S>;
+  using T = WgTile<KD, KH, KW, S, G>;
   constexpr int TAPS = T::TAPS, NT = 16 * NSUB, GS = pad_row16(NT);
   constexpr int R = 16 / PACK, CH = 16 * NPL + R, C4 = CH / 4;
   constexpr int XS = CH == 20 ? 24 : CH;
@@ -926,7 +927,7 @@
     if (tile + 1 < t_end) prefetch(tile + 1);
 #pragma unroll 2
     for (int grp = 0; grp < T::TVOX / 4; ++grp) {
-      const int xq = grp & 3, ly = (grp >> 2) & 3, lz = grp >> 4;
+      const int xq = grp % T::XQ, ly = (grp / T::XQ) % T::TH, lz = grp / (T::XQ * T::TH);
       float b[NSUB], a[NPL][TPW], ap[TPP];
 #pragma unroll
       for (int nn = 0; nn < NSUB; ++nn) b[nn] = Gw[(grp * 4) * GS + nn * 16];
@@ -979,17 +980,19 @@
 
 struct WgPlan {
   int ntz, nty, ntx, ntiles, ncisub, ncot, nchunks, tiles_per_chunk, nsub, kslots;
+  int geom;
   const float* in_stats;
   int in_act;
   float in_slope;
 };
 
 
-template <int KD, int KH, int KW, int S>
+template <int KD, int KH, int KW, int S, int G = 0>
 WgPlan wgrad_plan(const CfunConv3dParams& p, int nsub) {
-  using T = WgTile<KD, KH, KW, S>;
+  using T = WgTile<KD, KH, KW, S, G>;
   WgPlan w;
   w.nsub = nsub;
+  w.geom = G;
   w.ntz = cdiv(p.Do, T::TD); w.nty = cdiv(p.Ho, T::TH); w.ntx = cdiv(p.Wo, T::TW);
   w.ntiles = p.N * w.ntz * w.nty * w.ntx;
   w.ncisub = (wgrad_fused_shape<KD, KH, KW, S>() && wgrad_fused_mode(p, nsub)) ? 1 : cdiv(p.Ci, 16);
@@ -1007,10 +1010,11 @@
   return w;
 }
 
-template <int KD, int KH, int KW, int S, int NSUB>
+template <int KD, int KH, int KW, int S, int NSUB, int G = 0>
 int launch_wgrad_mfma(const float* x, const float* g, float* partial, const CfunConv3dParams& p, const WgPlan& w,
                       hipStream_t st) {
-  using T = WgTile<KD, KH, KW, S>;
+  using T = WgTile<KD, KH, KW, S, G>;
+  if (w.geom != G) return CFUN_EINVAL;
   constexpr int NT = 16 * NSUB, GS = pad_row16(NT);
   const size_t lds = (size_t)(T::IVOX * T::XS + T::TVOX * GS) * sizeof(float) + 8 * sizeof(float4);
   const int64_t lim = (int64_t)1 << 31;
@@ -1022,9 +1026,9 @@
       const size_t ldsf = (size_t)(T::IVOX * xs + T::TVOX * GS) * sizeof(float) + 2 * (xs / 4) * sizeof(float4);
       const bool in = w.in_stats != nullptr || w.in_act != CFUN_ACT_NONE;
       void (*kf)(const float*, const float*, float*, CfunConv3dParams, int, int, int, int, int, int, WgIn) =
-          in ? k_wgrad_fused<KD, KH, KW, S, NSUB, 1, 4, true> : k_wgrad_fused<KD, KH, KW, S, NSUB, 1, 4, false>;
+          in ? k_wgrad_fused<KD, KH, KW, S, NSUB, 1, 4, true, G> : k_wgrad_fused<KD, KH, KW, S, NSUB, 1, 4, false, G>;
       if constexpr (S == 1) {
-        if ((mode & 15) == 2) kf = in ? k_wgrad_fused<KD, KH, KW, S, NSUB, 2, 2, true> : k_wgrad_fused<KD, KH, KW, S, NSUB, 2, 2, false>;
+        if ((mode & 15) == 2) kf = in ? k_wgrad_fused<KD, KH, KW, S, NSUB, 2, 2, true, G> : k_wgrad_fused<KD, KH, KW, S, NSUB, 2, 2, false, G>;
       }
       if (ldsf > 64 * 1024) {
         hipError_t e = hipFuncSetAttribute(reinterpret_cast<const void*>(kf), hipFuncAttributeMaxDynamicSharedMemorySize, (int)ldsf);
@@ -1037,21 +1041,21 @@
     }
   }
   const bool in = w.in_stats != nullptr || w.in_act != CFUN_ACT_NONE;
-  auto kern = k_wgrad_mfma<KD, KH, KW, S, NSUB, false, 1, false>;
+  auto kern = k_wgrad_mfma<KD, KH, KW, S, NSUB, false, 1, false, G>;
   auto pick = [&](auto in_c) {
     constexpr bool I = decltype(in_c)::value;
-    kern = k_wgrad_mfma<KD, KH, KW, S, NSUB, false, 1, I>;
+    kern = k_wgrad_mfma<KD, KH, KW, S, NSUB, false, 1, I, G>;
     if constexpr (KD * KH * KW == 27) {
       const int pack = w.ncisub > 1 ? 1 : p.Ci <= 4 ? 4 : p.Ci <= 8 ? 2 : 1;
       const bool ts = S == 1 && p.d2s && p.tap_skip;
       if constexpr (S == 1) {
-        if (ts) kern = pack == 4 ? k_wgrad_mfma<KD, KH, KW, S, NSUB, true, 4, I>
-                     : pack == 2 ? k_wgrad_mfma<KD, KH, KW, S, NSUB, true, 2, I>
-                                 : k_wgrad_mfma<KD, KH, KW, S, NSUB, true, 1, I>;
-      }
-      if (!ts) kern = pack == 4 ? k_wgrad_mfma<KD, KH, KW, S, NSUB, false, 4, I>
-                    : pack == 2 ? k_wgrad_mfma<KD, KH, KW, S, NSUB, false, 2, I>
-                                : k_wgrad_mfma<KD, KH, KW, S, NSUB, false, 1, I>;
+        if (ts) kern = pack == 4 ? k_wgrad_mfma<KD, KH, KW, S, NSUB, true, 4, I, G>
+                     : pack == 2 ? k_wgrad_mfma<KD, KH, KW, S, NSUB, true, 2, I, G>
+                                 : k_wgrad_mfma<KD, KH, KW, S, NSUB, true, 1, I, G>;
+      }
+      if (!ts) kern = pack == 4 ? k_wgrad_mfma<KD, KH, KW, S, NSUB, false, 4, I, G>
+                    : pack == 2 ? k_wgrad_mfma<KD, KH, KW, S, NSUB, false, 2, I, G>
+                                : k_wgrad_mfma<KD, KH, KW, S, NSUB, false, 1, I, G>;
     }
   };
   if (in) pick(std::true_type{}); else pick(std::false_type{});
@@ -1066,19 +1070,19 @@
   return CFUN_OK;
 }
 
-template <int KD, int KH, int KW, int S>
+template <int KD, int KH, int KW, int S, int G = 0>
 int dispatch_wgrad(const float* x, const float* g, float* partial, const CfunConv3dParams& p, const WgPlan& w,
                    hipStream_t st) {
   if constexpr (max_nsub<KD, KH, KW, S>() == 1) {
     if (w.nsub != 1) return CFUN_EINVAL;
-    return launch_wgrad_mfma<KD, KH, KW, S, 1>(x, g, partial, p, w, st);
+    return launch_wgrad_mfma<KD, KH, KW, S, 1, G>(x, g, partial, p, w, st);
   } else {
     switch (w.nsub) {
-      case 1: return launch_wgrad_mfma<KD, KH, KW, S, 1>(x, g, partial, p, w, st);
-      case 2: return launch_wgrad_mfma<KD, KH, KW, S, 2>(x, g, partial, p, w, st);
-      case 3: return launch_wgrad_mfma<KD, KH, KW, S, 3>(x, g, partial, p, w, st);
-      case 4: return launch_wgrad_mfma<KD, KH, KW, S, 4>(x, g, partial, p, w, st);
-      default: return launch_wgrad_mfma<KD, KH, KW, S, 5>(x, g, partial, p, w, st);
+      case 1: return launch_wgrad_mfma<KD, KH, KW, S, 1, G>(x, g, partial, p, w, st);
+      case 2: return launch_wgrad_mfma<KD, KH, KW, S, 2, G>(x, g, partial, p, w, st);
+      case 3: return launch_wgrad_mfma<KD, KH, KW, S, 3, G>(x, g, partial, p, w, st);
+      case 4: return launch_wgrad_mfma<KD, KH, KW, S, 4, G>(x, g, partial, p, w, st);
+      default: return launch_wgrad_mfma<KD, KH, KW, S, 5, G>(x, g, partial, p, w, st);
     }
   }
 }
@@ -1131,6 +1135,24 @@
 CFUN_MFMA_DECL_G8(k333s2)
 CFUN_MFMA_DECL_G8(k222s1)
 
+#define CFUN_WGRAD_DECL_G8(NAME)                                                                                    \
+  void cfun_mfma_wgrad_plan_g8_##NAME(const CfunConv3dParams& p, int nsub, cfun_mfma::WgPlan* w);                   \
+  int cfun_mfma_wgrad_g8_##NAME(const float* x, const float* g, float* partial, const CfunConv3dParams& p,          \
+                                const cfun_mfma::WgPlan& w, hipStream_t st);
+
+#define CFUN_WGRAD_DEFINE_G8(NAME, KD, KH, KW, S)                                                                   \
+  void cfun_mfma_wgrad_plan_g8_##NAME(const CfunConv3dParams& p, int nsub, cfun_mfma::WgPlan* w) {                  \
+    *w = cfun_mfma::wgrad_plan<KD, KH, KW, S, 1>(p, nsub);                                                          \
+  }                                                                                                                 \
+  int cfun_mfma_wgrad_g8_##NAME(const float* x, const float* g, float* partial, const CfunConv3dParams& p,          \
+                                const cfun_mfma::WgPlan& w, hipStream_t st) {                                       \
+    return cfun_mfma::dispatch_wgrad<KD, KH, KW, S, 1>(x, g, partial, p, w, st);                                    \
+  }
+
+CFUN_WGRAD_DECL_G8(k333s1)
+CFUN_WGRAD_DECL_G8(k333s2)
+CFUN_WGRAD_DECL_G8(k111s1)
+
 int cfun_tile_geom(const CfunConv3dParams* p, int g8_exists);
 
 CFUN_MFMA_DECL(k333s1)
diff --git a/cfun_amd/csrc/conv3d_wgrad_k111s1_g8.hip b/cfun_amd/csrc/conv3d_wgrad_k111s1_g8.hip
--- /dev/null
+++ b/cfun_amd/csrc/conv3d_wgrad_k111s1_g8.hip
@@ -0,0 +1,3 @@
+#include "conv3d_mfma.h"
+
+CFUN_WGRAD_DEFINE_G8(k111s1, 1, 1, 1, 1)
diff --git a/cfun_amd/csrc/conv3d_wgrad_k333s1_g8.hip b/cfun_amd/csrc/conv3d_wgrad_k333s1_g8.hip
--- /dev/null
+++ b/cfun_amd/csrc/conv3d_wgrad_k333s1_g8.hip
@@ -0,0 +1,3 @@
+#include "conv3d_mfma.h"
+
+CFUN_WGRAD_DEFINE_G8(k333s1, 3, 3, 3, 1)
diff --git a/cfun_amd/csrc/conv3d_wgrad_k333s2_g8.hip b/cfun_amd/csrc/conv3d_wgrad_k333s2_g8.hip
--- /dev/null
+++ b/cfun_amd/csrc/conv3d_wgrad_k333s2_g8.hip
@@ -0,0 +1,3 @@
+#include "conv3d_mfma.h"
+
+CFUN_WGRAD_DEFINE_G8(k333s2, 3, 3, 3, 2)
diff --git a/cfun_amd/csrc/conv3d_wino_wgrad.hip b/cfun_amd/csrc/conv3d_wino_wgrad.hip
--- a/cfun_amd/csrc/conv3d_wino_wgrad.hip
+++ b/cfun_amd/csrc/conv3d_wino_wgrad.hip
@@ -13,10 +13,21 @@
 constexpr int WG_GVOX = 2 * 4 * 16;
 constexpr int WG_XROW = 2 * WG_XH * 16;
 
-template <int NSUB, bool D2S>
-__global__ void __launch_bounds__(256)
+template <int G>
+struct WgGeom {
+  static constexpr int TH = G ? 8 : 4, TW = G ? 8 : 16;
+  static constexpr int IY = TH + 2, XH = TW / 2 + 1;
+  static constexpr int XROWS = 4 * IY, XVOX = XROWS * 2 * XH, XROW = 2 * XH * 16;
+  static constexpr int JP = TW / 2, QR = JP / 4;
+};
+static_assert(WgGeom<0>::IY == WG_IY && WgGeom<0>::XH == WG_XH && WgGeom<0>::XVOX == WG_XVOX && WgGeom<0>::XROW == WG_XROW, "G16");
+
+template <int NSUB, bool D2S, int G>
+__global__ void __launch_bounds__(256, (G == 1 && NSUB == 2 && !D2S) ? 3 : 1)
 k_wgrad_wino(const float* __restrict__ x, const float* __restrict__ g, float* __restrict__ partial, CfunConv3dParams p,
              int ntz, int nty, int ntx, int ncisub, int ncot, int tiles_per_chunk, int ntiles) {
+  using W = WgGeom<G>;
+  constexpr int WG_IY = W::IY, WG_XH = W::XH, WG_XVOX = W::XVOX, WG_XROW = W::XROW, JP = W::JP, QR = W::QR;
   constexpr int NT = 16 * NSUB, GS = cfun_mfma::pad_row16(NT);
   constexpr int X_ITEMS = WG_XVOX * 4, X_LOADS = cdiv(X_ITEMS, 256);
   constexpr int G_ITEMS = WG_GVOX * (NT / 4), G_LOADS = cdiv(G_ITEMS, 256);
@@ -45,7 +56,7 @@
     const int ty = t % nty; t /= nty;
     const int tz = t % ntz;
     const int n = t / ntz;
-    const int z0 = tz * 2, y0 = ty * 4, x0 = tx * 16;
+    const int z0 = tz * 2, y0 = ty * W::TH, x0 = tx * W::TW;
     xvalid = 0; gvalid = 0;
 #pragma unroll
     for (int i = 0; i < X_LOADS; ++i) {
@@ -62,8 +73,8 @@
     for (int i = 0; i < G_LOADS; ++i) {
       const int it = tid + i * 256;
       const int slot = it / (NT / 4), col = (it % (NT / 4)) * 4;
-      const int j = slot & 7, par = (slot >> 3) & 1, lrow = slot >> 4;
-      const int oz = z0 + (lrow >> 2), oy = y0 + (lrow & 3), ox = x0 + 2 * j + par;
+      const int j = slot % JP, par = (slot / JP) & 1, lrow = slot / (2 * JP);
+      const int oz = z0 + lrow / W::TH, oy = y0 + lrow % W::TH, ox = x0 + 2 * j + par;
       bool ok = (it < G_ITEMS) & (cobase + col < p.Co) & (oz < p.Do) & (oy < p.Ho) & (ox < p.Wo);
       unsigned off;
       if (D2S) {
@@ -115,13 +126,13 @@
     if (tile + 1 < t_end) prefetch(tile + 1);
 #pragma unroll 1
     for (int grp = 0; grp < 16; ++grp) {
-      const int lrow = grp >> 1, q = grp & 1;
-      const int hrow = (lrow >> 2) * WG_IY + (lrow & 3);
+      const int lrow = grp / QR, q = grp % QR;
+      const int hrow = (lrow / W::TH) * WG_IY + lrow % W::TH;
       float b[NSUB], a[9];
 #pragma unroll
       for (int nn = 0; nn < NSUB; ++nn) {
-        const float* gp = Gw + ((lrow * 2) * 8 + q * 4) * GS + nn * 16;
-        b[nn] = ce * gp[0] + cg * gp[8 * GS];
+        const float* gp = Gw + ((lrow * 2) * JP + q * 4) * GS + nn * 16;
+        b[nn] = ce * gp[0] + cg * gp[JP * GS];
       }
       const float* x1 = Xa1 + hrow * WG_XROW + q * 64;
       const float* x2 = Xa2 + hrow * WG_XROW + q * 64;
@@ -335,13 +346,25 @@
 }
 
 struct WgPlanW {
-  int nsub, ntz, nty, ntx, ntiles, ncisub, ncot, nchunks, tiles_per_chunk;
+  int nsub, ntz, nty, ntx, ntiles, ncisub, ncot, nchunks, tiles_per_chunk, geom;
 };
+
+int wino_wgrad_2d(const CfunConv3dParams& p);
+
+int wino_wgrad_nsub(const CfunConv3dParams& p) {
+  return p.CoP <= 16 ? 1 : ((p.CoP + 31) / 32 * 32 < (p.CoP + 47) / 48 * 48 ? 2 : 3);
+}
+
+int wino_wgrad_geom(const CfunConv3dParams& p) {
+  if (wino_wgrad_2d(p)) return 0;
+  return cfun_tile_geom(&p, p.d2s && wino_wgrad_nsub(p) == 3 ? 2 : 1);
+}
 
 WgPlanW make_wg_plan(const CfunConv3dParams& p) {
   WgPlanW w;
-  w.nsub = p.CoP <= 16 ? 1 : ((p.CoP + 31) / 32 * 32 < (p.CoP + 47) / 48 * 48 ? 2 : 3);
-  w.ntz = cdiv(p.Do, 2); w.nty = cdiv(p.Ho, 4); w.ntx = cdiv(p.Wo, 16);
+  w.geom = wino_wgrad_geom(p);
+  w.nsub = wino_wgrad_nsub(p);
+  w.ntz = cdiv(p.Do, 2); w.nty = cdiv(p.Ho, w.geom ? 8 : 4); w.ntx = cdiv(p.Wo, w.geom ? 8 : 16);
   w.ntiles = p.N * w.ntz * w.nty * w.ntx;
   w.ncisub = cdiv(p.Ci, 16);
   w.ncot = cdiv(p.CoP, 16 * w.nsub);
@@ -390,13 +413,13 @@
   return CFUN_OK;
 }
 
-template <int NSUB>
+template <int NSUB, int G>
 int launch_wg(const float* x, const float* g, float* partial, const CfunConv3dParams& p, const WgPlanW& w, hipStream_t st) {
   constexpr int GS = cfun_mfma::pad_row16(16 * NSUB);
-  size_t lds = (size_t)(WG_XVOX * 16 + WG_GVOX * GS) * sizeof(float);
+  size_t lds = (size_t)(WgGeom<G>::XVOX * 16 + WG_GVOX * GS) * sizeof(float);
   const size_t scratch = (size_t)4 * 16 * 16 * NSUB * sizeof(float);
   if (lds < scratch) lds = scratch;
-  auto kern = p.d2s ? k_wgrad_wino<NSUB, true> : k_wgrad_wino<NSUB, false>;
+  auto kern = p.d2s ? k_wgrad_wino<NSUB, true, G> : k_wgrad_wino<NSUB, false, G>;
   if (lds > 64 * 1024) {
     hipError_t e = hipFuncSetAttribute(reinterpret_cast<const void*>(kern), hipFuncAttributeMaxDynamicSharedMemorySize, (int)lds);
     if (e != hipSuccess) return (int)e;
@@ -422,6 +445,8 @@
   if (p->d2s) return 0;
   return !(p->Ci <= 8 || (p->Ci > 16 && p->Ci <= 20));
 }
+
+int cfun_wino_wgrad_geom(const CfunConv3dParams* p) { return wino_wgrad_geom(*p); }
 
 size_t cfun_wino_wgrad_workspace_bytes(const CfunConv3dParams* p) {
   const WgPlanW w = make_wg_plan(*p);
@@ -438,9 +463,16 @@
       default: return launch_wg2<3>(x, g, ws, *p, w, st);
     }
   }
+  if (w.geom) {
+    switch (w.nsub) {
+      case 1: return launch_wg<1, 1>(x, g, ws, *p, w, st);
+      case 2: return launch_wg<2, 1>(x, g, ws, *p, w, st);
+      default: return launch_wg<3, 1>(x, g, ws, *p, w, st);
+    }
+  }
   switch (w.nsub) {
-    case 1: return launch_wg<1>(x, g, ws, *p, w, st);
-    case 2: return launch_wg<2>(x, g, ws, *p, w, st);
-    default: return launch_wg<3>(x, g, ws, *p, w, st);
-  }
-}
+    case 1: return launch_wg<1, 0>(x, g, ws, *p, w, st);
+    case 2: return launch_wg<2, 0>(x, g, ws, *p, w, st);
+    default: return launch_wg<3, 0>(x, g, ws, *p, w, st);
+  }
+}
diff --git a/include/cfun_tile.h b/include/cfun_tile.h
--- a/include/cfun_tile.h
+++ b/include/cfun_tile.h
@@ -9,6 +9,8 @@
 
 int cfun_conv3d_fwd_tile(const CfunConv3dParams* p, int32_t out[3]);
 
+int cfun_conv3d_wgrad_tile(const CfunConv3dParams* p, int32_t out[3]);
+
 #ifdef __cplusplus
 }
 #endif
```

Result: faster. 26.28 volumes/s, median of 6 (+1.3%).
